# victordeleau/MUI-DeepAutoEncoder

Hardware: AMD Instinct MI355X
Metric: training samples/sec at 3x512-dim input, batch 8192 (higher is better)
Workload: dtype bf16; 1 GPU; embedding.yaml topology: 3 slots x 512 (io 1536), z=io, 4+4 layers -> 10 x Linear(1536,1536); batch 8192 rows per GPU, Adam lr 1e-5 wd 1e-4 clip 1.0, slot-blanking k=1; global_batch=8192, parallelism=dp1

## Files before the change

include/codae_hip.h:

```cpp
#ifndef CODAE_HIP_H
#define CODAE_HIP_H

#include <stddef.h>
#include <stdint.h>

#ifdef __cplusplus
extern "C" {
#endif

#define CODAE_ABI_VERSION 11

enum {
    CODAE_OK = 0,
    CODAE_E_INVALID = -1,
    CODAE_E_HIP = -2,
    CODAE_E_UNSUPPORTED = -3
};

enum {
    CODAE_PREC_F32 = 0,
    CODAE_PREC_BF16 = 1
};

enum {
// ... 150 lines not shown
    float max_grad_norm;
    int32_t step;
    float loss_scale_rows;
} codae_hyper;

const char* codae_last_error(void);
int codae_abi_version(void);
#define CODAE_N_STRUCTS 7
int codae_struct_sizes(int32_t* out, int32_t capacity);
int codae_reload_env(void);

int codae_create(const codae_spec* spec, codae_handle* out);
int codae_destroy(codae_handle h);
int codae_get_sizes(codae_handle h, codae_sizes* out);
int codae_param_offsets(codae_handle h, int32_t layer, int64_t* w_off, int64_t* b_off, int64_t* shadow_off);

int codae_forward(codae_handle h, const codae_buffers* bufs, const float* x, float* y, int32_t B,
                  int32_t layer_lo, int32_t layer_hi, int32_t save_for_backward, void* stream);
int codae_backward(codae_handle h, const codae_buffers* bufs, const float* dy, float* dx, int32_t B,
                   int32_t layer_lo, int32_t layer_hi, void* stream);
int codae_sync_shadows(codae_handle h, const codae_buffers* bufs, void* stream);

int codae_step_forward_loss(codae_handle h, const codae_buffers* bufs, const codae_batch* batch,
                            const codae_hyper* hyper, float* out_y, void* stream);
int codae_step_backward(codae_handle h, const codae_buffers* bufs, int32_t B, int32_t layer_lo,
                        int32_t layer_hi, void* stream);
int codae_step_update(codae_handle h, const codae_buffers* bufs, const codae_hyper* hyper, void* stream);
int codae_train_step_graph(codae_handle h, const codae_buffers* bufs, const codae_batch* batch,
                           const codae_hyper* hyper, void* stream);
int codae_step_backward_async(codae_handle h, const codae_buffers* bufs, int32_t B, int32_t layer_lo,
                              int32_t layer_hi, void* stream);
int codae_side_stream(codae_handle h, void** stream_out);
int codae_join(codae_handle h, void* stream);

int codae_span_sumsq(const float* g, int64_t n, double* acc, void* stream);
int codae_step_update_span(codae_handle h, const codae_buffers* bufs, const codae_hyper* hyper, int64_t lo, int64_t hi,
                           const double* total_sq, void* stream);
int codae_sync_transposed(codae_handle h, const codae_buffers* bufs, void* stream);
int codae_train_step(codae_handle h, const codae_buffers* bufs, const codae_batch* batch,
                     const codae_hyper* hyper, void* stream);
int codae_dp_unique_id(void* out, int32_t capacity);
int codae_dp_init(codae_handle h, const void* unique_id, int32_t rank, int32_t world);
int codae_dp_destroy(codae_handle h);
int codae_train_step_dp(codae_handle h, const codae_buffers* bufs, const codae_batch* batch, const codae_hyper* hyper,
                        int32_t n_buckets, const int32_t* bucket_lo, const int32_t* bucket_hi, void* stream);
int codae_step_path(codae_handle h, const codae_buffers* bufs, int32_t B);
int codae_set_input_noise(codae_handle h, const codae_noise* noise);
int codae_set_loss_emphasis(codae_handle h, const codae_emphasis* emphasis);
int codae_set_recon_loss(codae_handle h, const codae_recon_loss* loss);
int codae_set_hidden_dropout(codae_handle h, const codae_dropout* d);
int codae_set_slot_contrast(codae_handle h, const codae_slot_contrast* contrast);
int codae_set_optimizer(codae_handle h, const codae_optimizer* opt);
int codae_set_slot_presence(codae_handle h, const uint8_t* present, int64_t n_rows, int32_t n_slots);
int codae_set_tied_weights(codae_handle h, int32_t on);
int codae_graph_captures(codae_handle h);
int codae_eval_step(codae_handle h, const codae_buffers* bufs, const codae_batch* batch, float* out_y,
                    void* stream);

enum {
    CODAE_K_GEMM_FWD = 0,
    CODAE_K_GEMM_DGRAD = 1,
    CODAE_K_GEMM_WGRAD = 2,
    CODAE_K_LOSS = 3,
    CODAE_K_GATHER = 4,
    CODAE_K_SUMSQ = 5,
    CODAE_K_ADAM = 6,
    CODAE_K_SLAB_REDUCE = 7,
    CODAE_K_CHAIN = 8,
    CODAE_K_BIAS_FINISH = 9,
    CODAE_K_DROPOUT = 10,
    CODAE_K_COUNT = 11
};
int codae_profile_begin(codae_handle h, uint32_t class_mask, int32_t max_records);
int codae_profile_stride(codae_handle h, int32_t every_n_steps);
int codae_profile_end(codae_handle h, int32_t* kinds, float* ms, int32_t capacity, int32_t* n_out);

int codae_corrupt(const float* x, const float* mask, float* out, int64_t n, void* stream);
int codae_corrupt_batch(const codae_batch* batch, const codae_noise* noise, int32_t step, const int32_t* noise_rows, void* out,
                        int32_t out_bf16, int64_t out_ld, void* stream);
int codae_emph_loss(const codae_batch* batch, const codae_noise* noise, int32_t step, const codae_emphasis* emphasis, const float* y,
                    void* dy, int32_t dy_bf16, int64_t dy_ld, float inv_n, float* colsum_part, double* parts, void* stream);
int codae_emph_loss_blocks(int32_t B);
int codae_recon_loss_fwd_bwd(const codae_batch* batch, const codae_noise* noise, int32_t step, const codae_emphasis* emphasis,
                             const codae_recon_loss* loss, const float* y, void* dy, int32_t dy_bf16, int64_t dy_ld, float inv_n,
                             float* colsum_part, double* parts, void* stream);
int codae_recon_loss_blocks(int32_t B);
int64_t codae_slot_contrast_ws_bytes(int32_t n_slots, int32_t n_neg, int32_t E, int32_t bf16);
int codae_slot_contrast_prepare(const float* data, int32_t io, const codae_slot_contrast* contrast, int32_t step, int32_t bf16, void* stream);
int codae_slot_contrast_fwd_bwd(const codae_batch* batch, const codae_noise* noise, int32_t step, const codae_emphasis* emphasis,
                                const codae_slot_contrast* contrast, const float* y, void* dy, int32_t dy_bf16, int64_t dy_ld, float scale,
                                float* colsum_part, double* parts, void* stream);
int codae_slot_contrast_blocks(int32_t B);
int codae_corrupt_batch_present(const codae_batch* batch, const codae_noise* noise, int32_t step, const int32_t* noise_rows, void* out,
                                int32_t out_bf16, int64_t out_ld, const uint8_t* present, int32_t n_slots, void* stream);
int codae_mse_loss_present(const codae_batch* batch, const float* y, void* dy, int32_t dy_bf16, int64_t dy_ld, float inv_n,
                           float* colsum_part, double* parts, const uint8_t* present, int32_t n_slots, void* stream);
int codae_emph_loss_present(const codae_batch* batch, const codae_noise* noise, int32_t step, const codae_emphasis* emphasis, const float* y,
                            void* dy, int32_t dy_bf16, int64_t dy_ld, float inv_n, float* colsum_part, double* parts,
                            const uint8_t* present, int32_t n_slots, void* stream);
int codae_recon_loss_fwd_bwd_present(const codae_batch* batch, const codae_noise* noise, int32_t step, const codae_emphasis* emphasis,
                                     const codae_recon_loss* loss, const float* y, void* dy, int32_t dy_bf16, int64_t dy_ld, float inv_n,
                                     float* colsum_part, double* parts, const uint8_t* present, int32_t n_slots, void* stream);
int codae_slot_contrast_prepare_present(const float* data, int32_t io, const codae_slot_contrast* contrast, int32_t step, int32_t bf16,
                                        const uint8_t* present, int32_t n_slots, void* stream);
int codae_slot_contrast_fwd_bwd_present(const codae_batch* batch, const codae_noise* noise, int32_t step, const codae_emphasis* emphasis,
                                        const codae_slot_contrast* contrast, const float* y, void* dy, int32_t dy_bf16, int64_t dy_ld,
// ... 26 lines not shown
                             const int32_t* var_size, const int32_t* var_type, const float* undo_scale, const float* undo_min,
                             const int32_t* mask_id, const uint8_t* mask_table, const int32_t* k_of_mask, int32_t k_max,
                             double* acc, void* stream);
int codae_row_norms(const float* m, int64_t rows, int32_t E, float* out, void* stream);
int codae_ranking_loss(const float* pred, const float* fmask, const int32_t* idx, int32_t B, int32_t io, int32_t n_slots,
                       int32_t E, const float* inventory, const float* inventory_norm, int64_t n_obs, const int32_t* val_idx,
                       int32_t n_val, double* out, void* stream);

int codae_ranking_loss_batched(const float* pred, int32_t B, int32_t io, int32_t n_slots, int32_t E, const int32_t* row_idx,
                               const int32_t* mask_id, const int32_t* mask_to_use, int32_t nb_run, int32_t run,
                               const uint8_t* mask_table, const float* inventory, const float* inventory_norm, int64_t n_obs,
                               const float* inv_val, const float* inv_val_norm, const int32_t* val_pos, const int32_t* val_group,
                               int32_t n_val, float* work, int32_t chunk, void* row_state, int32_t* perm_ws, float* q_ws, double* out,
                               void* stream);
int codae_gather_inventory_rows(const float* inventory, int64_t n_obs, int32_t E, int32_t n_slots, const int32_t* val_idx,
                                int32_t n_val, float* dst, void* stream);

int codae_topk_init(void* state, int32_t B, int32_t k, void* stream);
int codae_topk_merge(const float* scores, int64_t ld, int32_t rows, int32_t n, int32_t col0, int32_t k, const int32_t* row_map,
                     const int32_t* skip_col, void* state, void* stream);
int codae_topk_finish(const void* state, int32_t B, int32_t k, const int32_t* cand_row_id, int32_t* out_idx, float* out_score,
                      void* stream);
int codae_complete_topk(const float* pred, int32_t B, int32_t io, int32_t n_slots, int32_t E, const int32_t* slot,
                        const int32_t* row_idx, const int32_t* mask_id, const int32_t* mask_to_use, int32_t nb_run, int32_t run,
                        const uint8_t* mask_table, const float* cand, const float* cand_norm, const int32_t* cand_row_id,
                        int32_t n_cand, const int32_t* cand_count, const int32_t* exclude, const int32_t* cand_pos, int64_t n_obs,
                        int32_t k, float* work, int32_t chunk, void* row_state, int32_t* perm_ws, float* q_ws, void* topk_state,
                        int32_t* out_idx, float* out_score, void* stream);

int codae_linear_f32(const float* x, const float* W, const float* b, float* y, int32_t M, int32_t N,
                     int32_t K, int32_t relu, void* stream);
int codae_dgrad_f32(const float* dy, const float* W, const float* relu_src, float* dx, int32_t M,
                    int32_t N, int32_t K, void* stream);
int codae_wgrad_f32(const float* dy, const float* x, float* dW, float* db, int32_t M, int32_t N,
                    int32_t K, void* stream);
int codae_linear_bf16(const void* x, const void* W, const float* b, void* y, int32_t y_f32, int32_t M,
                      int32_t N, int32_t K, int32_t relu, void* stream);
int codae_dgrad_bf16(const void* dy, const void* W, const void* relu_src, void* dx, float* db_prev, float* db_ws,
                     int32_t M, int32_t N, int32_t K, void* stream);
int codae_wgrad_bf16(const void* dy, const void* x, float* dW, void* slabs, int64_t slab_bytes,
                     int32_t M, int32_t N, int32_t K, void* stream);
int codae_linear_act_f32(const float* x, const float* W, const float* b, float* y, int32_t M, int32_t N, int32_t K,
                         int32_t act, float p0, float p1, float p2, void* stream);
int codae_dgrad_act_f32(const float* dy, const float* W, const float* act_src, float* dx, int32_t M, int32_t N, int32_t K,
                        int32_t act, float p0, float p1, float p2, void* stream);
int codae_linear_act_bf16(const void* x, const void* W, const float* b, void* y, int32_t y_f32, int32_t M, int32_t N,
                          int32_t K, int32_t act, float p0, float p1, float p2, void* stream);
int codae_dgrad_act_bf16(const void* dy, const void* W, const void* act_src, void* dx, float* db_prev, float* db_ws,
                         int32_t M, int32_t N, int32_t K, int32_t act, float p0, float p1, float p2, void* stream);
int codae_debug_gemm_timeline(uint64_t* host_out, int32_t n_wg);
#define CODAE_GEMM_PLAN_FIELDS 15
int codae_debug_gemm_bf16_plan(const int32_t* desc, int32_t* out, int32_t capacity);
int codae_cast_f32_to_bf16(const float* src, void* dst, int64_t n, void* stream);
int codae_transpose_bf16(const void* src, void* dst, int32_t rows, int32_t cols, void* stream);

#ifdef __cplusplus
}
#endif
#endif
```

mui-deepautoencoder_amd/codae/hip/__init__.py:

```python
import ctypes as C
import os

_HERE = os.path.dirname(os.path.abspath(__file__))
LIB_PATH = os.environ.get("CODAE_HIP_LIB") or os.path.join(_HERE, "libcodae_hip.so")

PREC_F32 = 0
PREC_BF16 = 1

ABI_VERSION = 11
S_SQ_FULL, S_SQ_PARTIAL, S_GRAD_SQ, S_LAST_LOSS, S_STEP_SQ, S_CLIP_COEF = 0, 1, 2, 3, 4, 5
S_GRAD_SQ_SLOTS, S_N_SLOTS, S_ADAM_STEP, S_COUNT = 8, 64, 72, 80
ACT_NONE, ACT_RELU, ACT_LEAKY, ACT_RELU6, ACT_ELU, ACT_SOFTPLUS, ACT_HARDSIGMOID = 0, 1, 2, 3, 4, 5, 6
NOISE_NONE, NOISE_GAUSSIAN, NOISE_MASKING, NOISE_SALT_PEPPER = 0, 1, 2, 3
LOSS_MSE, LOSS_L1, LOSS_SMOOTH_L1, LOSS_HUBER, LOSS_SLOT_COSINE = 0, 1, 2, 3, 4
OPT_ADAM, OPT_ADAMW, OPT_SGD = 0, 1, 2
SCHED_CONSTANT, SCHED_COSINE, SCHED_LINEAR, SCHED_STEP = 0, 1, 2, 3
KERNEL_CLASSES = ("gemm_fwd", "gemm_dgrad", "gemm_wgrad", "loss", "gather", "sumsq", "adam", "slab_reduce", "chain",
                  "bias_finish", "dropout")


class HipError(RuntimeError):
    pass


# ... 53 lines not shown

class Optimizer(C.Structure):
    _fields_ = [("kind", C.c_int32), ("amsgrad", C.c_int32), ("momentum", C.c_float), ("nesterov", C.c_int32), ("sched", C.c_int32),
                ("warmup", C.c_int32), ("total", C.c_int32), ("period", C.c_int32), ("min_factor", C.c_float), ("gamma", C.c_float),
                ("vmax", C.c_void_p)]


class TiePair(C.Structure):
    _fields_ = [("enc_off", C.c_int64), ("dec_off", C.c_int64), ("rows", C.c_int32), ("cols", C.c_int32)]


class Dropout(C.Structure):
    _fields_ = [("p", C.POINTER(C.c_float)), ("n", C.c_int32), ("seed", C.c_uint64)]


_P, _I32, _I64, _F = C.c_void_p, C.c_int32, C.c_int64, C.c_float

PROTOTYPES = {
    "codae_last_error": (C.c_char_p, []),
    "codae_abi_version": (C.c_int, []),
    "codae_struct_sizes": (C.c_int, [C.POINTER(C.c_int32), _I32]),
    "codae_reload_env": (C.c_int, []),
    "codae_create": (C.c_int, [C.POINTER(Spec), C.POINTER(_P)]),
    "codae_destroy": (C.c_int, [_P]),
    "codae_get_sizes": (C.c_int, [_P, C.POINTER(Sizes)]),
    "codae_param_offsets": (C.c_int, [_P, _I32, C.POINTER(_I64), C.POINTER(_I64), C.POINTER(_I64)]),
    "codae_forward": (C.c_int, [_P, C.POINTER(Buffers), _P, _P, _I32, _I32, _I32, _I32, _P]),
    "codae_backward": (C.c_int, [_P, C.POINTER(Buffers), _P, _P, _I32, _I32, _I32, _P]),
    "codae_sync_shadows": (C.c_int, [_P, C.POINTER(Buffers), _P]),
    "codae_step_forward_loss": (C.c_int, [_P, C.POINTER(Buffers), C.POINTER(Batch), C.POINTER(Hyper), _P, _P]),
    "codae_step_backward": (C.c_int, [_P, C.POINTER(Buffers), _I32, _I32, _I32, _P]),
    "codae_step_update": (C.c_int, [_P, C.POINTER(Buffers), C.POINTER(Hyper), _P]),
    "codae_step_backward_async": (C.c_int, [_P, C.POINTER(Buffers), _I32, _I32, _I32, _P]),
    "codae_side_stream": (C.c_int, [_P, C.POINTER(C.c_void_p)]),
    "codae_profile_stride": (C.c_int, [_P, _I32]),
    "codae_join": (C.c_int, [_P, _P]),
    "codae_span_sumsq": (C.c_int, [_P, _I64, _P, _P]),
    "codae_step_update_span": (C.c_int, [_P, C.POINTER(Buffers), C.POINTER(Hyper), _I64, _I64, _P, _P]),
    "codae_sync_transposed": (C.c_int, [_P, C.POINTER(Buffers), _P]),
    "codae_train_step": (C.c_int, [_P, C.POINTER(Buffers), C.POINTER(Batch), C.POINTER(Hyper), _P]),
    "codae_train_step_graph": (C.c_int, [_P, C.POINTER(Buffers), C.POINTER(Batch), C.POINTER(Hyper), _P]),
    "codae_set_input_noise": (C.c_int, [_P, C.POINTER(Noise)]),
    "codae_set_loss_emphasis": (C.c_int, [_P, C.POINTER(Emphasis)]),
    "codae_set_recon_loss": (C.c_int, [_P, C.POINTER(ReconLoss)]),
    "codae_set_hidden_dropout": (C.c_int, [_P, C.POINTER(Dropout)]),
    "codae_set_slot_contrast": (C.c_int, [_P, C.POINTER(SlotContrast)]),
    "codae_set_optimizer": (C.c_int, [_P, C.POINTER(Optimizer)]),
    "codae_optimizer_update": (C.c_int, [_P, _P, _P, _P, _P, _I64, C.POINTER(Hyper), C.POINTER(Optimizer), _P, _P]),
    "codae_graph_captures": (C.c_int, [_P]),
    "codae_set_tied_weights": (C.c_int, [_P, _I32]),
    "codae_tie_fold": (C.c_int, [_P, C.POINTER(TiePair), _I32, _P]),
    "codae_tie_mirror": (C.c_int, [_P, _P, _P, C.POINTER(TiePair), _I32, _P]),
    "codae_set_slot_presence": (C.c_int, [_P, _P, _I64, _I32]),
    "codae_corrupt_batch_present": (C.c_int, [C.POINTER(Batch), C.POINTER(Noise), _I32, _P, _P, _I32, _I64, _P, _I32, _P]),
    "codae_mse_loss_present": (C.c_int, [C.POINTER(Batch), _P, _P, _I32, _I64, _F, _P, _P, _P, _I32, _P]),
    "codae_emph_loss_present": (C.c_int, [C.POINTER(Batch), C.POINTER(Noise), _I32, C.POINTER(Emphasis), _P, _P, _I32, _I64, _F, _P, _P,
                                          _P, _I32, _P]),
    "codae_recon_loss_fwd_bwd_present": (C.c_int, [C.POINTER(Batch), C.POINTER(Noise), _I32, C.POINTER(Emphasis), C.POINTER(ReconLoss), _P,
                                                   _P, _I32, _I64, _F, _P, _P, _P, _I32, _P]),
    "codae_slot_contrast_prepare_present": (C.c_int, [_P, _I32, C.POINTER(SlotContrast), _I32, _I32, _P, _I32, _P]),
    "codae_slot_contrast_fwd_bwd_present": (C.c_int, [C.POINTER(Batch), C.POINTER(Noise), _I32, C.POINTER(Emphasis),
                                                      C.POINTER(SlotContrast), _P, _P, _I32, _I64, _F, _P, _P, _P, _I32, _P]),
    "codae_slot_contrast_ws_bytes": (_I64, [_I32, _I32, _I32, _I32]),
    "codae_slot_contrast_prepare": (C.c_int, [_P, _I32, C.POINTER(SlotContrast), _I32, _I32, _P]),
    "codae_slot_contrast_fwd_bwd": (C.c_int, [C.POINTER(Batch), C.POINTER(Noise), _I32, C.POINTER(Emphasis), C.POINTER(SlotContrast), _P, _P,
                                              _I32, _I64, _F, _P, _P, _P]),
    "codae_slot_contrast_blocks": (C.c_int, [_I32]),
    "codae_dropout_fwd": (C.c_int, [_P, _I32, _I64, _I32, _I32, _P, _I32, _I32, _F, C.c_uint64, _P]),
    "codae_dropout_bwd": (C.c_int, [_P, _I32, _I64, _I32, _I32, _P, _I32, _I32, _F, C.c_uint64, _P, _P]),
    "codae_dropout_blocks": (C.c_int, [_I32]),
    "codae_emph_loss": (C.c_int, [C.POINTER(Batch), C.POINTER(Noise), _I32, C.POINTER(Emphasis), _P, _P, _I32, _I64, _F, _P, _P, _P]),
    "codae_emph_loss_blocks": (C.c_int, [_I32]),
    "codae_recon_loss_fwd_bwd": (C.c_int, [C.POINTER(Batch), C.POINTER(Noise), _I32, C.POINTER(Emphasis), C.POINTER(ReconLoss), _P, _P, _I32, _I64,
                                           _F, _P, _P, _P]),
    "codae_recon_loss_blocks": (C.c_int, [_I32]),
    "codae_corrupt_batch": (C.c_int, [C.POINTER(Batch), C.POINTER(Noise), _I32, _P, _P, _I32, _I64, _P]),
    "codae_noise_box_muller": (C.c_int, [_P, _P, _P, _P, _P, _I64, _P]),
    "codae_eval_step": (C.c_int, [_P, C.POINTER(Buffers), C.POINTER(Batch), _P, _P]),
    "codae_profile_begin": (C.c_int, [_P, C.c_uint32, _I32]),
    "codae_profile_end": (C.c_int, [_P, C.POINTER(C.c_int32), C.POINTER(C.c_float), _I32, C.POINTER(C.c_int32)]),
    "codae_corrupt": (C.c_int, [_P, _P, _P, _I64, _P]),
    "codae_expand_masks": (C.c_int, [_P, _P, _P, _I32, _I32, _I32, _P, _P, _P]),
    "codae_mse_loss_fwd_bwd": (C.c_int, [_P, _P, _P, _P, _I64, _F, _P, _P]),
    "codae_clip_adam": (C.c_int, [_P, _P, _P, _P, _I64, C.POINTER(Hyper), _P, _P]),
    "codae_combined_loss_fwd_bwd": (C.c_int, [_P, _P, _I32, _I32, _I32, _P, _P, _P, _P, _P, _P, _P, _P]),
    "codae_combined_loss_full": (C.c_int, [_P, _P, _I32, _I32, _I32, _P, _P, _P, _P, _P]),
    "codae_row_norms": (C.c_int, [_P, _I64, _I32, _P, _P]),
    "codae_ranking_loss": (C.c_int, [_P, _P, _P, _I32, _I32, _I32, _I32, _P, _P, _I64, _P, _I32, _P, _P]),
    "codae_ranking_loss_batched": (C.c_int, [_P, _I32, _I32, _I32, _I32, _P, _P, _P, _I32, _I32, _P, _P, _P, _I64, _P, _P, _P, _P, _I32, _P,
                                             _I32, _P, _P, _P, _P, _P]),
    "codae_dp_unique_id": (C.c_int, [_P, _I32]),
    "codae_dp_init": (C.c_int, [_P, _P, _I32, _I32]),
    "codae_dp_destroy": (C.c_int, [_P]),
    "codae_train_step_dp": (C.c_int, [_P, C.POINTER(Buffers), C.POINTER(Batch), C.POINTER(Hyper), _I32, _P, _P, _P]),
    "codae_monitor_accumulate": (C.c_int, [_P, _P, _I32, _I32, _I32, _P, _P, _P, _P, _P, _P, _P, _P, _I32, _P, _P]),
    "codae_gather_inventory_rows": (C.c_int, [_P, _I64, _I32, _I32, _P, _I32, _P, _P]),
    "codae_topk_init": (C.c_int, [_P, _I32, _I32, _P]),
    "codae_topk_merge": (C.c_int, [_P, _I64, _I32, _I32, _I32, _I32, _P, _P, _P, _P]),
    "codae_topk_finish": (C.c_int, [_P, _I32, _I32, _P, _P, _P, _P]),
    "codae_complete_topk": (C.c_int, [_P, _I32, _I32, _I32, _I32, _P, _P, _P, _P, _I32, _I32, _P, _P, _P, _P, _I32, _P, _P, _P, _I64,
                                      _I32, _P, _I32, _P, _P, _P, _P, _P, _P, _P]),
    "codae_step_path": (C.c_int, [_P, _P, _I32]),
    "codae_linear_f32": (C.c_int, [_P, _P, _P, _P, _I32, _I32, _I32, _I32, _P]),
    "codae_dgrad_f32": (C.c_int, [_P, _P, _P, _P, _I32, _I32, _I32, _P]),
    "codae_wgrad_f32": (C.c_int, [_P, _P, _P, _P, _I32, _I32, _I32, _P]),
    "codae_linear_bf16": (C.c_int, [_P, _P, _P, _P, _I32, _I32, _I32, _I32, _I32, _P]),
    "codae_dgrad_bf16": (C.c_int, [_P, _P, _P, _P, _P, _P, _I32, _I32, _I32, _P]),
    "codae_wgrad_bf16": (C.c_int, [_P, _P, _P, _P, _I64, _I32, _I32, _I32, _P]),
    "codae_linear_act_f32": (C.c_int, [_P, _P, _P, _P, _I32, _I32, _I32, _I32, _F, _F, _F, _P]),
    "codae_dgrad_act_f32": (C.c_int, [_P, _P, _P, _P, _I32, _I32, _I32, _I32, _F, _F, _F, _P]),
    "codae_linear_act_bf16": (C.c_int, [_P, _P, _P, _P, _I32, _I32, _I32, _I32, _I32, _F, _F, _F, _P]),
    "codae_dgrad_act_bf16": (C.c_int, [_P, _P, _P, _P, _P, _P, _I32, _I32, _I32, _I32, _F, _F, _F, _P]),
    "codae_cast_f32_to_bf16": (C.c_int, [_P, _P, _I64, _P]),
    "codae_debug_gemm_timeline": (C.c_int, [_P, _I32]),
    "codae_debug_gemm_bf16_plan": (C.c_int, [_P, _P, _I32]),
    "codae_transpose_bf16": (C.c_int, [_P, _P, _I32, _I32, _P]),
}

_lib = None


def lib():
    global _lib
    if _lib is not None:
        return _lib
    if not os.path.exists(LIB_PATH):
        raise HipError(
            "libcodae_hip.so is missing (%s). Build it with `python -c \"import __graft_entry__ as g; "
            "g.build()\"` or `make -C mui-deepautoencoder_amd/csrc`. There is no CPU fallback." % LIB_PATH)
    import torch
    handle = C.CDLL(LIB_PATH, mode=C.RTLD_GLOBAL)
    for name, (res, args) in PROTOTYPES.items():
        fn = getattr(handle, name)
        fn.restype = res
        fn.argtypes = args
    if handle.codae_abi_version() != ABI_VERSION:
        raise HipError("libcodae_hip.so ABI version %d, this binding is written for %d: rebuild the library"
                       % (handle.codae_abi_version(), ABI_VERSION))
    check_struct_sizes(handle)
    _lib = handle
    return _lib


def struct_sizes_expected():
    return [C.sizeof(Spec), C.sizeof(Sizes), C.sizeof(Buffers), C.sizeof(Batch), C.sizeof(Hyper), S_COUNT,
            len(KERNEL_CLASSES)]


def check_struct_sizes(handle):
    n = 7
    got = (C.c_int32 * n)()
    rc = handle.codae_struct_sizes(got, n)
    if rc != 0:
        raise HipError("codae_struct_sizes failed (%d)" % rc)
    want = struct_sizes_expected()
    names = ("codae_spec", "codae_sizes", "codae_buffers", "codae_batch", "codae_hyper", "CODAE_S_COUNT", "CODAE_K_COUNT")
    bad = ["%s: library %d, binding %d" % (nm, g, w) for nm, g, w in zip(names, list(got), want) if g != w]
    if bad:
        raise HipError("libcodae_hip.so and its ctypes binding disagree: " + "; ".join(bad))


def check(rc):
    if rc != 0:
        msg = lib().codae_last_error()
        raise HipError("codae_hip error %d: %s" % (rc, msg.decode() if msg else "?"))

# ... 9 lines not shown
```

mui-deepautoencoder_amd/codae/hip/engine.py:

```python
import ctypes as C

import torch

from . import (PREC_BF16, PREC_F32, S_COUNT, S_GRAD_SQ, S_GRAD_SQ_SLOTS, S_LAST_LOSS, S_N_SLOTS, S_SQ_FULL, S_SQ_PARTIAL,
               Batch, Buffers, Dropout, Emphasis,
               HipError, Hyper, Sizes, Spec, TiePair, check, current_stream, lib, ptr)


def precision_code(precision):
    if precision in (PREC_F32, "f32", "fp32", "parity"):
        return PREC_F32
    if precision in (PREC_BF16, "bf16", "throughput"):
        return PREC_BF16
    raise ValueError("unknown precision %r (use 'f32' or 'bf16')" % (precision,))


def _tie_pair_array(pairs):
    arr = (TiePair * max(len(pairs), 1))()
    for i, (e, d, r, c) in enumerate(pairs):
        arr[i] = TiePair(int(e), int(d), int(r), int(c))
    return arr


def tie_fold(grads, pairs):
# ... 28 lines not shown
        self.max_batch = int(max_batch)
        self.precision = precision_code(precision)
        ins = (C.c_int32 * self.L)(*[s[0] for s in self.schedule])
        outs = (C.c_int32 * self.L)(*[s[1] for s in self.schedule])
        relu = (C.c_uint8 * self.L)(*[1 if s[2] else 0 for s in self.schedule])
        self.activation = self._layer_acts(activation)
        spec = Spec(self.L, ins, outs, relu, self.max_batch, self.precision)
        if self.activation is not None:
            spec.act_kind = (C.c_uint8 * self.L)(*[a[0] for a in self.activation])
            spec.act_param = (C.c_float * (3 * self.L))(*[float(p) for a in self.activation for p in a[1:]])
        h = C.c_void_p()
        check(self._lib.codae_create(C.byref(spec), C.byref(h)))
        self._h = h
        sz = Sizes()
        check(self._lib.codae_get_sizes(self._h, C.byref(sz)))
        self.n_param = int(sz.n_param)
        with torch.cuda.device(device):
            f32 = dict(dtype=torch.float32, device=device)
            self._params = torch.zeros(self.n_param, **f32)
            self.grads = torch.zeros(self.n_param, **f32)
            self.adam_m = torch.zeros(self.n_param, **f32) if with_optimizer_state else None
            self.adam_v = torch.zeros(self.n_param, **f32) if with_optimizer_state else None
            self.shadow = (torch.zeros(int(sz.n_weight), dtype=torch.bfloat16, device=device)
                           if sz.n_weight > 0 else None)
            self.shadow_t = (torch.zeros(int(sz.n_weight), dtype=torch.bfloat16, device=device)
                             if sz.n_weight > 0 else None)
            self.acts = torch.zeros(max(int(sz.act_bytes), 16), dtype=torch.uint8, device=device)
            self.dacts = torch.zeros(max(int(sz.dact_bytes), 16), dtype=torch.uint8, device=device)
            self.slabs = (torch.zeros(int(sz.slab_bytes), dtype=torch.uint8, device=device)
                          if sz.slab_bytes > 0 else None)
            self.bias_parts = torch.zeros(max(int(sz.bias_part_bytes) // 4, 16), dtype=torch.float32, device=device)
            if int(sz.n_scalars) != S_COUNT:
                raise HipError("library reports %d scalars, binding expects %d" % (int(sz.n_scalars), S_COUNT))
            self.scalars = torch.zeros(int(sz.n_scalars), dtype=torch.float64, device=device)
        self.bufs = Buffers(ptr(self._params), ptr(self.grads), ptr(self.adam_m), ptr(self.adam_v), ptr(self.shadow),
                            ptr(self.acts), ptr(self.dacts), ptr(self.slabs), ptr(self.scalars), ptr(self.shadow_t),
                            ptr(self.bias_parts))
        self.w_off, self.b_off = [], []
        for l in range(self.L):
            w, b, s = C.c_int64(), C.c_int64(), C.c_int64()
            check(self._lib.codae_param_offsets(self._h, l, C.byref(w), C.byref(b), C.byref(s)))
            self.w_off.append(w.value)
            self.b_off.append(b.value)
        self.input_noise = None
        self.loss_emphasis = None
        self._emph_weights = None
        self.hidden_dropout = None
        self.recon_loss = None
        self.slot_contrast = None
        self._contrast_pins = None
        self.slot_presence = None
        self._presence_table = None
        self.tied_weights = False
        self.optimizer = None
        self.adam_vmax = None
        self.step_count = 0
        self.generation = 0

    def _layer_acts(self, activation):
        if activation is None:
            return None
        if isinstance(activation, (list, tuple)) and len(activation) == self.L and all(
                isinstance(a, (list, tuple)) for a in activation):
            acts = [tuple(a) for a in activation]
        else:
            if isinstance(activation, (list, tuple)):
                one = tuple(activation)
            else:
                from ..model.activation import from_factory
                one = from_factory(activation)
            acts = [one if s[2] else (0, 0.0, 0.0, 0.0) for s in self.schedule]
        for a in acts:
            if len(a) != 4:
                raise HipError("activation per layer must be (kind, p0, p1, p2), got %r" % (a,))
        return [(int(a[0]), float(a[1]), float(a[2]), float(a[3])) for a in acts]

    def __del__(self):
        h = getattr(self, "_h", None)
        if h is not None and h.value:
            try:
                self._lib.codae_destroy(h)
            except Exception:
                pass
            self._h = None

    def join(self):
        with torch.cuda.device(self.device):
            check(self._lib.codae_join(self._h, current_stream()))

    @property
    def params(self):
        self.join()
        return self._params

    def _view(self, flat, l, bias):
        self.join()
        k, n, _ = self.schedule[l]
        if bias:
            return flat[self.b_off[l]:self.b_off[l] + n]
        return flat[self.w_off[l]:self.w_off[l] + n * k].view(n, k)

    def weight(self, l): return self._view(self._params, l, False)
    def bias(self, l): return self._view(self._params, l, True)
    def weight_grad(self, l): return self._view(self.grads, l, False)
    def bias_grad(self, l): return self._view(self.grads, l, True)

# ... 89 lines not shown
    def _set_recon_struct(self, st):
        check(self._lib.codae_set_recon_loss(self._h, None if st is None else C.byref(st)))

    def set_slot_contrast(self, contrast, data=None, n_slots=None):
        if contrast is not None and not hasattr(contrast, "candidate_rows"):
            raise HipError("set_slot_contrast: expected a codae.tool.SlotContrast or None, got %r" % (contrast,))
        if contrast is None or contrast.is_default:
            self._set_contrast_struct(None)
            self.slot_contrast, self._contrast_pins = contrast, None
            return
        if data is None or data.dtype != torch.float32 or not data.is_contiguous() or data.device != self.device or data.dim() != 2:
            raise HipError("set_slot_contrast: data must be the contiguous fp32 [N, io] dataset on %s" % self.device)
        io = self.schedule[-1][1]
        if int(data.shape[1]) != io:
            raise HipError("set_slot_contrast: data has %d columns, the model %d" % (int(data.shape[1]), io))
        S = contrast._check_slots(n_slots, io)
        N = int(data.shape[0])
        contrast.check_rows(N)
        with torch.cuda.device(self.device):
            pool = None if contrast.candidates is None else torch.from_numpy(contrast.candidates).to(self.device)
            ids = None
            if contrast.distinct:
                from ..tool.contrast import item_ids
                ids = item_ids(data, S).to(torch.int32).contiguous()
            need = int(self._lib.codae_slot_contrast_ws_bytes(S, contrast.negatives, io // S, int(self.precision == PREC_BF16)))
            if need < 0:
                raise HipError("set_slot_contrast: no work space for S = %d, K = %d, E = %d" % (S, contrast.negatives, io // S))
            ws = torch.empty(need, dtype=torch.uint8, device=self.device)
        self._set_contrast_struct(contrast.as_struct(S, N, pool, ids, ws))
        self.slot_contrast, self._contrast_pins = contrast, (data, pool, ids, ws)

    def _set_contrast_struct(self, st):
        with torch.cuda.device(self.device):
            check(self._lib.codae_set_slot_contrast(self._h, None if st is None else C.byref(st)))

    def set_slot_presence(self, presence):
        if presence is not None and not hasattr(presence, "assign_masks"):
            raise HipError("set_slot_presence: expected a codae.tool.SlotPresence or None, got %r" % (presence,))
        if presence is None or presence.is_default:
            self._set_presence_table(None)
            self.slot_presence, self._presence_table = presence, None
            return
        table = presence.to(self.device)
        self._set_presence_table(table)
        self.slot_presence, self._presence_table = presence, table

    def _set_presence_table(self, table, n_rows=None, n_slots=None):
        if table is None:
            check(self._lib.codae_set_slot_presence(self._h, None, 0, 0))
            return
        check(self._lib.codae_set_slot_presence(self._h, ptr(table), int(table.shape[0]) if n_rows is None else int(n_rows),
                                                int(table.shape[1]) if n_slots is None else int(n_slots)))

    def set_optimizer(self, optimizer):
        if optimizer is not None and not hasattr(optimizer, "lr_at"):
            raise HipError("set_optimizer: expected a codae.tool.Optimizer or None, got %r" % (optimizer,))
        if optimizer is None or optimizer.is_default:
            self._set_optimizer_struct(None)
            self.optimizer = optimizer
            return
        vmax = self.adam_vmax
        if optimizer.amsgrad and vmax is None:
            with torch.cuda.device(self.device):
                vmax = torch.zeros(self.n_param, dtype=torch.float32, device=self.device)
        self._set_optimizer_struct(optimizer.as_struct(ptr(vmax)))
        self.optimizer, self.adam_vmax = optimizer, vmax

    def _set_optimizer_struct(self, st):
        check(self._lib.codae_set_optimizer(self._h, None if st is None else C.byref(st)))

    def set_tied_weights(self, on):
        on = bool(on)
        check(self._lib.codae_set_tied_weights(self._h, 1 if on else 0))
        self.tied_weights = on
        if on:
            self.sync_shadows()

    def tie_pairs(self):
        from ..tool.tied import TiedWeights
        return TiedWeights.flat_pairs(self.schedule, self.w_off)

    def graph_captures(self):
        return int(self._lib.codae_graph_captures(self._h))

    def set_hidden_dropout(self, dropout):
        if dropout is not None and not hasattr(dropout, "per_layer"):
            raise HipError("set_hidden_dropout: expected a codae.tool.HiddenDropout or None, got %r" % (dropout,))
        self._set_dropout_values(None if dropout is None else dropout.per_layer(self.L), 0 if dropout is None else dropout.seed)
        self.hidden_dropout = dropout

    def _set_dropout_values(self, p, seed=0):
        st = None
        if p is not None:
            arr = (C.c_float * max(len(p), 1))(*[float(v) for v in p])
            st = Dropout(arr, len(p), int(seed))
        check(self._lib.codae_set_hidden_dropout(self._h, None if st is None else C.byref(st)))

    def train_step(self, batch, hyper, graph=False):
        fn = self._lib.codae_train_step_graph if graph else self._lib.codae_train_step
        with torch.cuda.device(self.device):
            check(fn(self._h, C.byref(self.bufs), C.byref(batch), C.byref(hyper), current_stream()))
        self.step_count += 1

    def dp_unique_id(self):
        buf = (C.c_char * 128)()
        check(self._lib.codae_dp_unique_id(buf, 128))
# ... 104 lines not shown
```

mui-deepautoencoder_amd/codae/train.py:

```python
import torch

from .hostcpu import fit_host_threads, host_cpu_share
from .hip import HipError


class SubsetEpochSampler:

    def __init__(self, indices, batch_size):
        self.indices = torch.as_tensor(list(indices), dtype=torch.long)
        self.batch_size = int(batch_size)

    def __len__(self):
        return (len(self.indices) + self.batch_size - 1) // self.batch_size

    def _epoch_order(self):
        torch.empty((), dtype=torch.int64).random_()
        n_threads = torch.get_num_threads()
        if n_threads > 1:
            torch.set_num_threads(1)
        try:
            perm = torch.randperm(len(self.indices))
        finally:
            if n_threads > 1:
                torch.set_num_threads(n_threads)
        return self.indices[perm]

    def __iter__(self):
        order = self._epoch_order()
        for o in range(0, len(order), self.batch_size):
            yield order[o:o + self.batch_size]

    def device_batches(self, device, dtype=torch.int32):
        order = self._epoch_order().to(dtype)
        if torch.device(device).type == "cuda":
            st = getattr(self, "_stage", None)
            if st is None or st[0].numel() != order.numel() or st[0].dtype != order.dtype or st[1].device != torch.device(device):
                st = (torch.empty(order.numel(), dtype=order.dtype).pin_memory(), torch.empty(order.numel(), dtype=order.dtype, device=device),
                      torch.cuda.Event())
                self._stage = st
            else:
                st[2].synchronize()
            st[0].copy_(order)
            st[1].copy_(st[0], non_blocking=True)
            st[2].record()
            order = st[1]
        else:
            order = order.to(device)
        for o in range(0, len(order), self.batch_size):
            yield order[o:o + self.batch_size]


def shard_batch(batch_indices, rank, world):
# ... 202 lines not shown
        self.last_grad_sq = acc
        if hasattr(eng, "record_grad_sq"):
            eng.record_grad_sq(acc)
        for lo, hi in self.buckets:
            a, b = self._shard_bounds(lo, hi)
            eng.step_update_span(hyper, a, b, acc)
        eng.step_update_span(hyper, eng.b_off[0], eng.n_param, acc)
        in_place = self.dist.get_backend(self.group) == "nccl"
        works = []
        for t in eng.replica_tensors():
            for lo, hi in self.buckets:
                a, b = self._weight_span_bounds(lo, hi)
                sa, sb = self._shard_bounds(lo, hi)
                src = t[sa:sb] if in_place else t[sa:sb].clone()
                works.append(self.dist.all_gather_into_tensor(t[a:b], src, group=self.group, async_op=True))
        for w in works:
            w.wait()
        eng.after_replica_sync()
        eng.step_count += 1

    def gather_params(self):
        if not self.sharded or self.world == 1:
            return
        eng = self.engine
        p = eng.params if not hasattr(eng, "_params") else eng._params
        for lo, hi in self.buckets:
            a, b = self._weight_span_bounds(lo, hi)
            sa, sb = self._shard_bounds(lo, hi)
            self.dist.all_gather_into_tensor(p[a:b], p[sa:sb].clone(), group=self.group)

    def broadcast_params(self, params_flat):
        if self.world > 1:
            self.dist.broadcast(params_flat, src=0, group=self.group)

    def reduce_scalars(self, t):
        if self.world > 1:
            self.dist.all_reduce(t, op=self.dist.ReduceOp.SUM, group=self.group)
        return t


class _ResidentInventory:

    def __init__(self, data, S, E):
        self.nb_used_category, self.embedding_size = S, E
        self.data_per_category = {c: data[:, c * E:(c + 1) * E] for c in range(S)}


class HipEmbeddingTrainer:

    def __init__(self, schedule, data, mask_table_u8, mask_to_use_i32, lr, weight_decay, clip=1.0,
                 max_batch=8192, precision="bf16", device="cuda:0", distributed=False, n_buckets=None, use_graph=False,
                 sharded_update=False, native_dp=False, activation=None, n_slots=None, input_noise=None,
                 loss_emphasis=None, hidden_dropout=None, criterion=None, contrast=None, optimizer=None, presence=None,
                 tied_weights=None):
        from .hip.engine import DaeEngine
        fit_host_threads()
        self.device = torch.device(device)
        self.engine = DaeEngine(schedule, max_batch, precision, self.device, activation=activation)
        if input_noise is not None:
            self.engine.set_input_noise(input_noise)
        self.data = data.to(device=self.device, dtype=torch.float32).contiguous()
        self.mask_table = None if mask_table_u8 is None else mask_table_u8.to(self.device).contiguous()
        self.mask_to_use = None if mask_to_use_i32 is None else mask_to_use_i32.to(self.device).contiguous()
        self.lr, self.weight_decay, self.clip = lr, weight_decay, clip
        self.n_slots = n_slots
        if loss_emphasis is not None:
            self.set_loss_emphasis(loss_emphasis)
        if hidden_dropout is not None:
            self.set_hidden_dropout(hidden_dropout)
        if criterion is not None:
            self.set_criterion(criterion)
        if contrast is not None:
            self.set_contrast(contrast)
        if optimizer is not None:
            self.set_optimizer(optimizer)
        self.presence = None
        if presence is not None:
            self.set_presence(presence)
        if tied_weights:
            self.set_tied_weights(True)
        self.dp = DataParallel(self.engine, n_buckets=n_buckets, sharded=sharded_update, native=native_dp) if distributed else None
        self.world = self.dp.world if self.dp else 1
        self.use_graph = bool(use_graph) and self.dp is None
        self._idx_buf = torch.zeros(max_batch, dtype=torch.int32, device=self.device) if self.use_graph else None
        self._mid_buf = torch.zeros(max_batch, dtype=torch.int32, device=self.device) if self.use_graph else None
        self._graph_stream = torch.cuda.Stream(device=self.device) if self.use_graph else None

    def set_loss_emphasis(self, emphasis):
        S = None
        if emphasis is not None and getattr(emphasis, "slot_weight", None) is not None and (self.n_slots or self.mask_table is not None):
            S = self._slots()[0]
        self.engine.set_loss_emphasis(emphasis, n_slots=S)

    def set_criterion(self, criterion):
        S = None
        if criterion is not None and getattr(criterion, "kind", None) == "slot_cosine":
            if not self.n_slots and self.mask_table is None:
                raise HipError("criterion slot_cosine: the trainer has neither n_slots nor a mask table to read the slots from; "
                               "construct it with n_slots")
            S = self._slots()[0]
        self.engine.set_recon_loss(criterion, n_slots=S)

    def set_contrast(self, contrast):
        S = None
        if contrast is not None and not getattr(contrast, "is_default", True):
            if not self.n_slots and self.mask_table is None:
                raise HipError("slot contrast: the trainer has neither n_slots nor a mask table to read the slots from; "
                               "construct it with n_slots")
            S = self._slots()[0]
        self.engine.set_slot_contrast(contrast, self.data, n_slots=S)

    def set_presence(self, presence):
        if presence is not None and not getattr(presence, "is_default", True) and presence.n_rows != int(self.data.shape[0]):
            raise HipError("slot presence: the table has %d rows, the dataset %d" % (presence.n_rows, int(self.data.shape[0])))
        self.engine.set_slot_presence(presence)
        self.presence = None if presence is None or presence.is_default else presence
        self.__dict__.pop("_retrievers", None)

    def set_tied_weights(self, on):
        dp = self.__dict__.get("dp")
        if on and dp is not None and dp.sharded and self.engine.L >= 2:
            from .tool.tied import TiedWeights
            raise TiedWeights.sharded_refusal(self.engine.L)
        self.engine.set_tied_weights(bool(on))

    def set_optimizer(self, optimizer):
        self.engine.set_optimizer(optimizer)

    def current_lr(self):
        opt = self.engine.optimizer
        if opt is None:
            from .tool.optimizer import Optimizer
            opt = Optimizer()
        return opt.lr_at(self.lr, self.engine.step_count + 1)

    def set_hidden_dropout(self, dropout):
        self.engine.set_hidden_dropout(dropout)

    def load_params(self, params):
# ... 129 lines not shown
```

mui-deepautoencoder_amd/csrc/codae_common.h:

```cpp
#pragma once
#include <hip/hip_runtime.h>
#include <stdint.h>
#include <stdio.h>
#include <type_traits>

#include "codae_hip.h"

namespace codae {

void set_error(const char* fmt, ...);

#define CODAE_HIP_CHECK(expr)                                                              \
    do {                                                                                   \
        hipError_t e_ = (expr);                                                            \
        if (e_ != hipSuccess) {                                                            \
            codae::set_error("%s failed: %s (%s:%d)", #expr, hipGetErrorString(e_), __FILE__, __LINE__); \
            return CODAE_E_HIP;                                                            \
        }                                                                                  \
    } while (0)

#define CODAE_LAUNCH_CHECK()                                                               \
    do {                                                                                   \
        hipError_t e_ = hipGetLastError();                                                 \
        if (e_ != hipSuccess) {                                                            \
// ... 129 lines not shown
        k0 += 0x9E3779B9u; k1 += 0xBB67AE85u;
    }
    return make_uint4(c0, c1, c2, c3);
}

struct PresArgs {
    const uint8_t* tab;
    int S, E;
};
template <int W>
__device__ __forceinline__ uint32_t present_bits(const PresArgs& p, int64_t row, const int* sl) {
    const uint8_t* __restrict__ t = p.tab + row * p.S;
    const uint32_t p0 = t[sl[0]] != 0 ? 1u : 0u;
    if (sl[W - 1] == sl[0]) return p0 ? ((1u << W) - 1u) : 0u;
    uint32_t bits = p0;
#pragma unroll
    for (int k = 1; k < W; ++k) bits |= (t[sl[k]] != 0 ? 1u : 0u) << k;
    return bits;
}
int check_presence(const uint8_t* present, int n_slots, int io, const char* who);

static inline int64_t round_up(int64_t x, int64_t m) { return (x + m - 1) / m * m; }

enum { STORE_PLAIN = 0, STORE_WT = 1 };
int store_policy_for(int64_t out_bytes);

template <int POL>
struct TileStore {
    __amdgpu_buffer_rsrc_t rsrc;
    __device__ __forceinline__ explicit TileStore(void* tile_base) {
        if constexpr (POL != STORE_PLAIN) rsrc = __builtin_amdgcn_make_buffer_rsrc(tile_base, 0, 0x7fffffff, 0x00020000);
    }
    __device__ __forceinline__ void store16(void* p, uint32_t byte_off, u32x4 v) const {
        if constexpr (POL == STORE_PLAIN) *reinterpret_cast<u32x4*>(p) = v;
        else __builtin_amdgcn_raw_buffer_store_b128(v, rsrc, (int)byte_off, 0, 16);
    }
};

struct EnvToggles {
    int gemm_tile = -1;
    int gemm_dbg = 0;
    int wgrad_splitk = 0;
    int small_tile_max = 200;
    int small_stages = 4;
    int f32_gemm = 0;
    int group_tile = -1;
    bool side_priority_set = false; int side_priority = 0;
    bool no_wt = false, single_stream = false, tail_on_side = false, no_fused_loss = false, flat_adam = false,
         no_fused_norm = false, no_chain = false, no_deep_small = false,
         no_relu_bits = false,
         no_prefetch = false,
         no_defer_wgrad = false;
    bool no_folded_loss_finish = false;
    int store_policy = -1;
};
const EnvToggles& env();
void env_reload();

struct GemmF32 {
    const float* A; int64_t a_rs, a_ks;
    const float* B; int64_t b_rs, b_ks;
    float* C; int64_t ldc;
    int M, N, K;
    const float* bias;
    int relu;
    const float* relu_src;
    int64_t ld_relu;
    float* colsum_part;
    const int* m_dev;
    int split_k;
    int act;
    float act_p[3];
};
int gemm_f32(const GemmF32& g, hipStream_t s);
int gemm_f32x3(const GemmF32& g, hipStream_t s);
bool gemm_f32x3_takes(const GemmF32& g);
inline int gemm_f32_colsum_rows(int M) { return (M + 63) / 64; }

constexpr int CODAE_GROUP_MAX = 16;
struct GemmF32Group {
    int n;
    GemmF32 g[CODAE_GROUP_MAX];
    int wg_begin[CODAE_GROUP_MAX + 1];
};
int gemm_f32x3_grouped(GemmF32Group& grp, hipStream_t s);

enum { OP_KC = 0,
       OP_KS = 1
};
struct LossFuse {
    int enabled;
    const float* data;
    const int32_t* row_idx;
    const int32_t* mask_id;
    const int32_t* mask_to_use;
    int nb_run, run;
    const uint8_t* table;
    int io;
    int B;
    float inv_n;
    double* parts;
};

struct GemmBf16 {
    const bf16_t* A; int64_t lda; int a_mode;
    const bf16_t* B; int64_t ldb; int b_mode;
// ... 1 lines not shown
    int M, N, K;
    const float* bias;
    int relu;
    const bf16_t* relu_src; int64_t ld_relu;
    float* colsum_part;
    int split_k;
    LossFuse loss;
    int dbg;
    uint8_t* relu_bits_out; const uint8_t* relu_bits; int64_t ld_bits;
    const void* prefetch; int64_t prefetch_bytes;
    int coscheduled;
    double* sumsq_slots;
    int act;
    float act_p[3];
    int store_policy;
};
bool gemm_bf16_supported(int M, int N, int K);

struct GemmTile { int bm, bn; };
constexpr GemmTile TILE_256x192{256, 192}, TILE_128x192{128, 192}, TILE_128x128{128, 128}, TILE_64x128{64, 128}, TILE_64x64{64, 64};
inline int ceil_div(int a, int b) { return (a + b - 1) / b; }
inline int tile_count(int M, int N, GemmTile t) { return ceil_div(M, t.bm) * ceil_div(N, t.bn); }

enum { BF16_ONE_BARRIER = 0,
       BF16_PIPELINED = 1,
       BF16_PIPELINED_ABL = 2
};
struct Bf16Plan {
    int family;
    int bm, bn;
    int stages;
    int loader;
    int epi;
    int dbg;
    int act;
    int store_policy;
    int tiles_m, tiles_n;
    int64_t workgroups;
};
Bf16Plan gemm_bf16_plan(const GemmBf16& g);
bool gemm_bf16_takes_relu_bits(int M, int N);
int gemm_bf16_colsum_rows(const GemmBf16& g);
int gemm_bf16_loss_parts(const GemmBf16& g);
int gemm_bf16(const GemmBf16& g, hipStream_t s);
int gemm_bf16_pipe(const GemmBf16& g, const Bf16Plan& plan, hipStream_t s);
int choose_split_k(int N, int K, int rows);

struct GemmBf16Group {
    int n;
    GemmBf16 g[CODAE_GROUP_MAX];
    int wg_begin[CODAE_GROUP_MAX + 1];
};
int gemm_bf16_grouped(GemmBf16Group& grp, hipStream_t s);
int gemm_bf16_pipe_grouped(GemmBf16Group& grp, hipStream_t s);

constexpr int CODAE_CHAIN_MAX_WIDTH = 512;
constexpr int CODAE_CHAIN_MAX_LAYERS = 16;
constexpr int CODAE_CHAIN_MAX_BIAS = 6144;
struct ChainArgs {
    int L, rows, B;
    int width[CODAE_CHAIN_MAX_LAYERS + 1];
    uint32_t relu_flags;
    double* scalars;
    const bf16_t* W[CODAE_CHAIN_MAX_LAYERS];
    const bf16_t* Wt[CODAE_CHAIN_MAX_LAYERS];
    const float* bias[CODAE_CHAIN_MAX_LAYERS];
    bf16_t* act[CODAE_CHAIN_MAX_LAYERS];
    bf16_t* dact[CODAE_CHAIN_MAX_LAYERS];
    float* colsum_part[CODAE_CHAIN_MAX_LAYERS];
    const float* data; const int32_t* row_idx; const int32_t* mask_id; const uint8_t* mask_table;
    const int32_t* mask_to_use; int nb_run, run;
    float inv_n;
    double* loss_parts;
    int do_backward;
};
bool chain_supported(int L, const int* in, const int* out);
int chain_rows_per_workgroup();
int launch_chain_step(const ChainArgs& a, hipStream_t s);

int launch_gather_corrupt(const codae_batch* b, void* out, int out_bf16, hipStream_t s, int64_t out_ld = 0, double* zero_norm = nullptr,
                          const uint8_t* present = nullptr, int n_slots = 0);
int check_noise(const codae_noise* noise);
int launch_gather_noise(const codae_batch* b, const codae_noise* noise, int32_t step, const double* step_dev, void* out,
                        int out_bf16, hipStream_t s, int64_t out_ld = 0, const int32_t* noise_rows = nullptr, double* zero_norm = nullptr,
                        const uint8_t* present = nullptr, int n_slots = 0);
int launch_noise_box_muller(const uint32_t* ra, const uint32_t* rb, float* rho, float* c, float* sn, int64_t n, hipStream_t s);
int launch_cast_bf16(const float* src, bf16_t* dst, int64_t n, hipStream_t s);
int launch_corrupt(const float* x, const float* mask, float* out, int64_t n, hipStream_t s);
int launch_expand_masks(const int32_t* mask_id, const uint8_t* table, const int32_t* k_of_mask, int B, int io,
                        int k_max, float* masks_out, float* fmask_out, hipStream_t s);
struct LossLaunch {
    const codae_batch* batch; const codae_noise* noise; int32_t step; const double* step_dev;
    const codae_emphasis* emph; const uint8_t* present; int n_slots;
    const float* y; void* dy; int dy_bf16; int64_t dy_ld; float scale ;
    float* colsum_part; double* parts;
};
inline int64_t loss_dy_ld(const LossLaunch& ll) { return ll.dy_ld > 0 ? ll.dy_ld : (ll.batch ? ll.batch->io : 0); }
int check_loss_launch(const char* who, const LossLaunch& ll, bool needs_dy);
int launch_mse_loss(const LossLaunch& ll, int want_grad, hipStream_t s);
int mse_loss_colsum_rows(int B);
int check_emphasis(const codae_emphasis* emph);
int launch_emph_loss(const LossLaunch& ll, hipStream_t s);
int launch_finish_emph_loss(double* scalars, double inv_n, hipStream_t s, const double* parts, int n_parts);
int check_recon_loss(const codae_recon_loss* loss, int io);
int launch_recon_loss(const LossLaunch& ll, const codae_recon_loss* loss, hipStream_t s);
int check_slot_contrast(const codae_slot_contrast* c, int io, int bf16);
int64_t slot_contrast_ws_bytes(int S, int K, int E, int bf16);
inline int slot_contrast_blocks(int B) { return (B + 31) / 32; }
int slot_contrast_warm();
int launch_slot_contrast_prepare(const float* data, int io, const codae_slot_contrast* c, int32_t step, const double* step_dev, int bf16,
                                 hipStream_t s, const uint8_t* present = nullptr, int n_slots = 0);
int launch_slot_contrast(const LossLaunch& ll, const codae_slot_contrast* c, hipStream_t s);
int launch_slot_contrast_finish(double* scalars, double scale, const double* parts, int n_parts, hipStream_t s);
int check_dropout_p(float p, const char* who);
inline int dropout_blocks(int B) { return (B + 63) / 64; }
int launch_dropout_fwd(void* a, int bf16, int64_t ld, int B, int width, const int32_t* row_idx, int layer, int32_t step,
                       const double* step_dev, float p, uint64_t seed, hipStream_t s);
int launch_dropout_bwd(void* d, int bf16, int64_t ld, int B, int width, const int32_t* row_idx, int layer, int32_t step,
                       const double* step_dev, float p, uint64_t seed, float* colsum_part, hipStream_t s);
int launch_mse_dense(const float* x, const float* y, const float* fmask, float* dy, int64_t n, float inv_n,
                     double* scalars, hipStream_t s);
int launch_sumsq(const float* g, int64_t n, double* out, hipStream_t s);
int launch_sumsq_to(const float* g, int64_t n, double* acc, hipStream_t s);
int launch_clip_coef(const double* total_sq, float max_norm, double* coef_out, hipStream_t s);
int launch_clip_adam(float* p, float* g, float* m, float* v, int64_t n, const codae_hyper* hp,
                     const double* grad_sq, bf16_t* shadow, const double* coef_in, hipStream_t s,
                     const double* step_dev = nullptr, const codae_optimizer* opt = nullptr, float* vmax = nullptr);
int check_optimizer(const codae_optimizer* o);
bool optimizer_is_default(const codae_optimizer* o);
codae_optimizer optimizer_canonical(const codae_optimizer* o);
int launch_set_scalar(double* dst, double value, hipStream_t s);
int launch_clip_adam_tiled(float* p, float* g, float* m, float* v, const codae_hyper* hp, const double* grad_sq,
                           bf16_t* shadow, bf16_t* shadow_t, int n_layers, const int64_t* w_off, const int* rows,
                           const int* cols, int transposed_from, int64_t bias_off, int64_t bias_n, hipStream_t s,
                           const double* step_dev = nullptr, const codae_optimizer* opt = nullptr, float* vmax = nullptr);
int launch_tie_fold(float* g, const codae_tie_pair* pairs, int n, hipStream_t s);
int launch_tie_mirror(float* p, bf16_t* shadow, bf16_t* shadow_t, const codae_tie_pair* pairs, int n, hipStream_t s);
int launch_transpose_bf16(const bf16_t* src, bf16_t* dst, int n, const int64_t* off, const int* rows, const int* cols,
                          hipStream_t s);
int gemm_bf16_timeline(unsigned long long* host_out, int n_wg);
int launch_reduce_slabs_epi(const float* slabs, int n_slabs, int64_t stride, int M, int N, float* C, int64_t ldc, const float* bias,
                            int relu, const float* relu_src, int64_t ld_relu, float* colsum_part, hipStream_t s,
                            int act = CODAE_ACT_NONE, const float* act_p = nullptr);
int launch_reduce_slabs(const float* slabs, int n_slabs, int64_t slab_stride, float* out, int64_t n, double* sumsq,
                        hipStream_t s);
int launch_finish_loss(double* scalars, double inv_n, hipStream_t s, const double* parts = nullptr, int n_parts = 0);
int launch_cast_f32(const bf16_t* src, float* dst, int64_t n, hipStream_t s);
int launch_colsum_f32(const float* src, int M, int N, float* out, hipStream_t s);
int launch_colsum_parts_f32(const float* src, int M, int N, float* parts, hipStream_t s);
struct BiasFinishJobs {
    int n;
    const float* parts[64];
    float* out[64];
    int rows[64], cols[64];
    int col_begin[65];
};
struct LossFinish { double* scalars; double inv_n; const double* parts; int n_parts; };
int launch_bias_finish(const BiasFinishJobs& jobs, double* sumsq, hipStream_t s, const LossFinish* loss = nullptr);

}
```

mui-deepautoencoder_amd/csrc/elementwise.hip:

```cpp
#include "loss_sweep.h"

namespace codae {
namespace {

constexpr int NT = 256;
static_assert(NT == LOSS_NT, "loss_sweep strides the columns by LOSS_NT threads");

inline int grid_for(int64_t work_items) {
    int64_t b = (work_items + NT - 1) / NT;
    if (b < 1) b = 1;
    if (b > 2048) b = 2048;
    return (int)b;
}

template <int W>
__device__ __forceinline__ void zero_absent(float* v, const PresArgs& pa, int64_t row, int c) {
    int sl[W];
    slots_of<W>(c, pa.E, sl);
    const uint32_t pb = present_bits<W>(pa, row, sl);
#pragma unroll
    for (int k = 0; k < W; ++k) v[k] = ((pb >> k) & 1u) ? v[k] : 0.f;
}

__device__ __forceinline__ void zero_norm_scalars(double* zero_norm) {
    if (zero_norm != nullptr && blockIdx.x == 0) {
        if (threadIdx.x == 0) zero_norm[CODAE_S_GRAD_SQ] = 0.0;
        if (threadIdx.x < CODAE_S_N_SLOTS) zero_norm[CODAE_S_GRAD_SQ_SLOTS + threadIdx.x] = 0.0;
    }
}

template <bool PRES>
__global__ __launch_bounds__(NT) void gather_corrupt_bf16x8_kernel(const float* __restrict__ data,
                                                                   const int32_t* __restrict__ row_idx,
                                                                   const int32_t* __restrict__ mask_id,
                                                                   const uint8_t* __restrict__ table, int B, int io,
                                                                   bf16_t* __restrict__ out,
                                                                   const int32_t* __restrict__ mask_to_use, int nb_run,
                                                                   int run, int64_t out_ld, double* zero_norm, PresArgs pa) {
    zero_norm_scalars(zero_norm);
    const bool masked = (mask_id != nullptr) || (mask_to_use != nullptr);
    const int cols = io / 8;
    const int64_t total = (int64_t)B * cols;
    for (int64_t e = (int64_t)blockIdx.x * NT + threadIdx.x; e < total; e += (int64_t)gridDim.x * NT) {
        const int b = (int)(e / cols);
        const int c = (int)(e - (int64_t)b * cols) * 8;
        const int64_t src_row = row_idx ? row_idx[b] : b;
        const float* src = data + src_row * io + c;
        const float4 x0 = *reinterpret_cast<const float4*>(src);
        const float4 x1 = *reinterpret_cast<const float4*>(src + 4);
        float v[8] = {x0.x, x0.y, x0.z, x0.w, x1.x, x1.y, x1.z, x1.w};
        if (masked) {
            const int id = mask_id ? mask_id[b] : mask_to_use[src_row * nb_run + run];
            const uint2 m = *reinterpret_cast<const uint2*>(table + (int64_t)id * io + c);
#pragma unroll
            for (int k = 0; k < 8; ++k) v[k] = (((k < 4 ? m.x : m.y) >> (8 * (k & 3))) & 0xff) ? v[k] : 0.f;
        }
        if constexpr (PRES) zero_absent<8>(v, pa, src_row, c);
        uint4 o;
        o.x = pack_bf16x2(v[0], v[1]); o.y = pack_bf16x2(v[2], v[3]);
        o.z = pack_bf16x2(v[4], v[5]); o.w = pack_bf16x2(v[6], v[7]);
        *reinterpret_cast<uint4*>(out + (int64_t)b * out_ld + c) = o;
    }
}

template <bool VEC, bool OUT_BF16, bool PRES>
__global__ __launch_bounds__(NT) void gather_corrupt_kernel(const float* __restrict__ data,
                                                            const int32_t* __restrict__ row_idx,
                                                            const int32_t* __restrict__ mask_id,
                                                            const uint8_t* __restrict__ table, int B, int io,
                                                            void* __restrict__ out,
                                                            const int32_t* __restrict__ mask_to_use, int nb_run,
                                                            int run, int64_t out_ld, double* zero_norm, PresArgs pa) {
    zero_norm_scalars(zero_norm);
    constexpr int W = VEC ? 4 : 1;
    const bool masked = (mask_id != nullptr) || (mask_to_use != nullptr);
    const int cols = io / W;
    const int64_t total = (int64_t)B * cols;
    for (int64_t e = (int64_t)blockIdx.x * NT + threadIdx.x; e < total; e += (int64_t)gridDim.x * NT) {
        const int b = (int)(e / cols);
        const int c = (int)(e - (int64_t)b * cols) * W;
        const int64_t src_row = row_idx ? row_idx[b] : b;
        const float* src = data + src_row * io + c;
        float v[4];
        if constexpr (VEC) {
            const float4 x = *reinterpret_cast<const float4*>(src);
            v[0] = x.x; v[1] = x.y; v[2] = x.z; v[3] = x.w;
            if (masked) {
                const int id = mask_id ? mask_id[b] : mask_to_use[src_row * nb_run + run];
                const uint32_t m = *reinterpret_cast<const uint32_t*>(table + (int64_t)id * io + c);
#pragma unroll
                for (int k = 0; k < 4; ++k) v[k] = ((m >> (8 * k)) & 0xff) ? v[k] : 0.f;
            }
        } else {
            v[0] = src[0];
            if (masked) {
                const int id = mask_id ? mask_id[b] : mask_to_use[src_row * nb_run + run];
                v[0] = table[(int64_t)id * io + c] ? v[0] : 0.f;
            }
        }
        if constexpr (PRES) zero_absent<W>(v, pa, src_row, c);
        const int64_t o = (int64_t)b * out_ld + c;
        if constexpr (OUT_BF16) {
            bf16_t* op = reinterpret_cast<bf16_t*>(out) + o;
            if constexpr (VEC) *reinterpret_cast<uint2*>(op) = pack_bf16x4(v[0], v[1], v[2], v[3]);
            else op[0] = f32_to_bf16(v[0]);
        } else {
            float* op = reinterpret_cast<float*>(out) + o;
            if constexpr (VEC) *reinterpret_cast<float4*>(op) = make_float4(v[0], v[1], v[2], v[3]);
            else op[0] = v[0];
        }
    }
}

// ... 660 lines not shown
        if (c0 + c < C && r0 + r8 < R) {
            bf16_t e[8];
#pragma unroll
            for (int k = 0; k < 8; ++k) e[k] = tile[r8 + k][c];
            uint4 v;
            v.x = (uint32_t)e[0] | ((uint32_t)e[1] << 16); v.y = (uint32_t)e[2] | ((uint32_t)e[3] << 16);
            v.z = (uint32_t)e[4] | ((uint32_t)e[5] << 16); v.w = (uint32_t)e[6] | ((uint32_t)e[7] << 16);
            *reinterpret_cast<uint4*>(D + (int64_t)(c0 + c) * R + r0 + r8) = v;
        }
    }
}

}

int check_presence(const uint8_t* present, int n_slots, int io, const char* who) {
    if (present == nullptr) return CODAE_OK;
    CODAE_REQUIRE(n_slots >= 1 && n_slots <= 128, "%s: slot presence takes 1 .. 128 slots, got %d", who, n_slots);
    CODAE_REQUIRE(io > 0 && io % n_slots == 0, "%s: slot presence: n_slots %d does not divide io %d", who, n_slots, io);
    return CODAE_OK;
}

int launch_gather_corrupt(const codae_batch* b, void* out, int out_bf16, hipStream_t s, int64_t out_ld, double* zero_norm,
                          const uint8_t* present, int n_slots) {
    if (out_ld <= 0) out_ld = b ? b->io : 0;
    CODAE_REQUIRE(b && b->data && out && b->B > 0 && b->io > 0, "gather_corrupt: bad batch");
    int prc = check_presence(present, n_slots, b->io, "gather_corrupt");
    if (prc) return prc;
    const PresArgs pa{present, n_slots, present ? b->io / n_slots : 0};
    const bool masked = b->mask_id || b->mask_to_use;
    CODAE_REQUIRE(!masked || b->mask_table, "gather_corrupt: mask ids without mask_table");
    CODAE_REQUIRE(!b->mask_to_use || b->mask_id || (b->nb_run > 0 && b->run >= 0 && b->run < b->nb_run),
                  "gather_corrupt: run %d outside [0, %d)", b->run, b->nb_run);
    const bool vec = (b->io % 4 == 0) && (out_ld % 4 == 0) && a16(b->data) && a16(out) && (!masked || (reinterpret_cast<uintptr_t>(b->mask_table) & 3) == 0);
    const int64_t items = (int64_t)b->B * (vec ? b->io / 4 : b->io);
    const int grid = grid_for(items);
    if (vec && out_bf16 && b->io % 8 == 0 && (!masked || (reinterpret_cast<uintptr_t>(b->mask_table) & 7) == 0)) {
#define GC8(P) hipLaunchKernelGGL((gather_corrupt_bf16x8_kernel<P>), dim3(grid_for(items / 2)), dim3(NT), 0, s, b->data, b->row_idx, b->mask_id, \
                                  b->mask_table, b->B, b->io, reinterpret_cast<bf16_t*>(out), b->mask_to_use, b->nb_run, b->run, out_ld, zero_norm, pa)
        if (present) GC8(true);
        else GC8(false);
#undef GC8
        CODAE_LAUNCH_CHECK();
        return CODAE_OK;
    }
#define GCP(V, O, P) hipLaunchKernelGGL((gather_corrupt_kernel<V, O, P>), dim3(grid), dim3(NT), 0, s, b->data, b->row_idx, \
                                    b->mask_id, b->mask_table, b->B, b->io, out, b->mask_to_use, b->nb_run, b->run, out_ld, zero_norm, pa)
#define GC(V, O) do { if (present) GCP(V, O, true); else GCP(V, O, false); } while (0)
    if (vec && out_bf16) GC(true, true);
    else if (vec) GC(true, false);
    else if (out_bf16) GC(false, true);
    else GC(false, false);
#undef GC
#undef GCP
    CODAE_LAUNCH_CHECK();
    return CODAE_OK;
}

int check_noise(const codae_noise* n) {
    if (n == nullptr || n->kind == CODAE_NOISE_NONE) return CODAE_OK;
    CODAE_REQUIRE(n->kind == CODAE_NOISE_GAUSSIAN || n->kind == CODAE_NOISE_MASKING || n->kind == CODAE_NOISE_SALT_PEPPER,
                  "input noise: unknown kind %d", n->kind);
    if (n->kind == CODAE_NOISE_GAUSSIAN) {
        CODAE_REQUIRE(finite_f(n->p0) && n->p0 >= 0.f, "input noise: sigma %g must be finite and >= 0", (double)n->p0);
        return CODAE_OK;
    }
    CODAE_REQUIRE(finite_f(n->p0) && n->p0 >= 0.f && n->p0 <= 1.f, "input noise: p %g outside [0, 1]", (double)n->p0);
    if (n->kind == CODAE_NOISE_SALT_PEPPER) {
        CODAE_REQUIRE(finite_f(n->p1), "input noise: lo %g is not finite", (double)n->p1);
        CODAE_REQUIRE(finite_f(n->p2), "input noise: hi %g is not finite", (double)n->p2);
    }
    return CODAE_OK;
}

int launch_gather_noise(const codae_batch* b, const codae_noise* noise, int32_t step, const double* step_dev, void* out, int out_bf16,
                        hipStream_t s, int64_t out_ld, const int32_t* noise_rows, double* zero_norm, const uint8_t* present, int n_slots) {
    if (noise == nullptr || noise->kind == CODAE_NOISE_NONE) {
        CODAE_REQUIRE(present == nullptr || noise_rows == nullptr, "gather_corrupt: a presence table with noise_rows needs an input noise kind");
        return launch_gather_corrupt(b, out, out_bf16, s, out_ld, zero_norm, present, n_slots);
    }
    int rc = check_noise(noise);
    if (rc) return rc;
    rc = check_presence(present, n_slots, b ? b->io : 0, "gather_corrupt");
    if (rc) return rc;
    const PresArgs pa{present, n_slots, present ? b->io / n_slots : 0};
    if (out_ld <= 0) out_ld = b ? b->io : 0;
    CODAE_REQUIRE(b && b->data && out && b->B > 0 && b->io > 0, "gather_corrupt: bad batch");
    const bool masked = b->mask_id || b->mask_to_use;
    CODAE_REQUIRE(!masked || b->mask_table, "gather_corrupt: mask ids without mask_table");
    CODAE_REQUIRE(!b->mask_to_use || b->mask_id || (b->nb_run > 0 && b->run >= 0 && b->run < b->nb_run),
                  "gather_corrupt: run %d outside [0, %d)", b->run, b->nb_run);
    NoiseArgs na{};
    na.key0 = (uint32_t)(noise->seed & 0xffffffffu); na.key1 = (uint32_t)(noise->seed >> 32);
    na.step = (uint32_t)step; na.step_dev = step_dev; na.rows = noise_rows; na.zero_norm = zero_norm;
    na.thresh = (uint64_t)floor((double)noise->p0 * 4294967296.0);
    na.p0 = noise->p0; na.p1 = noise->p1; na.p2 = noise->p2;
    const bool vec = (b->io % 4 == 0) && (out_ld % 4 == 0) && a16(b->data) && a16(out) && (!masked || (reinterpret_cast<uintptr_t>(b->mask_table) & 3) == 0);
    const int64_t items = (int64_t)b->B * (vec ? b->io / 4 : b->io);
    const int grid = grid_for(items);
    const bool x8 = vec && out_bf16 && b->io % 8 == 0 && (!masked || (reinterpret_cast<uintptr_t>(b->mask_table) & 7) == 0);
#define GN8P(K, P) hipLaunchKernelGGL((gather_noise_bf16x8_kernel<K, P>), dim3(grid_for(items / 2)), dim3(NT), 0, s, b->data, b->row_idx, b->mask_id, \
                                  b->mask_table, b->B, b->io, reinterpret_cast<bf16_t*>(out), b->mask_to_use, b->nb_run, b->run, out_ld, na, pa)
#define GNP(V, O, K, P) hipLaunchKernelGGL((gather_noise_kernel<V, O, K, P>), dim3(grid), dim3(NT), 0, s, b->data, b->row_idx, b->mask_id, \
                                       b->mask_table, b->B, b->io, out, b->mask_to_use, b->nb_run, b->run, out_ld, na, pa)
#define GN8(K) do { if (present) GN8P(K, true); else GN8P(K, false); } while (0)
#define GN(V, O, K) do { if (present) GNP(V, O, K, true); else GNP(V, O, K, false); } while (0)
#define GN_KIND(K)                           \
// ... 468 lines not shown
```

mui-deepautoencoder_amd/csrc/engine.hip:

```cpp
#include <stdarg.h>
#include <stdlib.h>
#include <string.h>

#include <cmath>
#include <vector>

#include "layer_gemm.h"
#include <dlfcn.h>
#include <rccl/rccl.h>

namespace codae {

static thread_local char g_err[512] = "";

void set_error(const char* fmt, ...) {
    va_list ap;
    va_start(ap, fmt);
    vsnprintf(g_err, sizeof(g_err), fmt, ap);
    va_end(ap);
}

static EnvToggles g_env;
static bool g_env_loaded = false;

void env_reload() {
    EnvToggles e;
    if (const char* t = getenv("CODAE_GEMM_TILE")) {
        switch (t[0]) { case 's': e.gemm_tile = 0; break; case 'q': e.gemm_tile = 3; break; case 'x': e.gemm_tile = 6; break; case 'm': e.gemm_tile = 7; break; default: break; }
    }
    if (const char* d = getenv("CODAE_GEMM_DBG")) e.gemm_dbg = atoi(d);
    if (const char* k = getenv("CODAE_WGRAD_SPLITK")) e.wgrad_splitk = atoi(k) > 0 ? atoi(k) : 0;
    if (const char* k = getenv("CODAE_GROUP_TILE")) e.group_tile = (k[0] >= '0' && k[0] <= '2') ? k[0] - '0' : -1;
    if (const char* pr = getenv("CODAE_SIDE_PRIORITY")) { e.side_priority_set = true; e.side_priority = atoi(pr); }
    e.no_wt = getenv("CODAE_NO_WT") != nullptr;
    e.single_stream = getenv("CODAE_SINGLE_STREAM") != nullptr;
    e.tail_on_side = getenv("CODAE_TAIL_ON_SIDE") != nullptr;
    e.no_fused_loss = getenv("CODAE_NO_FUSED_LOSS") != nullptr;
    e.flat_adam = getenv("CODAE_FLAT_ADAM") != nullptr;
    e.no_fused_norm = getenv("CODAE_NO_FUSED_NORM") != nullptr;
    e.no_chain = getenv("CODAE_NO_CHAIN") != nullptr;
    e.no_deep_small = getenv("CODAE_NO_DEEP_SMALL") != nullptr;
    e.no_defer_wgrad = getenv("CODAE_NO_DEFER_WGRAD") != nullptr;
    e.no_prefetch = getenv("CODAE_NO_PREFETCH") != nullptr;
    e.no_relu_bits = getenv("CODAE_NO_RELU_BITS") != nullptr;
    e.no_folded_loss_finish = getenv("CODAE_NO_FOLDED_LOSS_FINISH") != nullptr;
    if (const char* k = getenv("CODAE_STORE_POLICY"))
        e.store_policy = !strcmp(k, "plain") ? STORE_PLAIN : (!strcmp(k, "wt") ? STORE_WT : -1);
    if (const char* k = getenv("CODAE_F32_GEMM")) e.f32_gemm = k[0] == 'n' ? 1 : (k[0] == 'x' ? 2 : 0);
    if (const char* k = getenv("CODAE_SMALL_TILE_MAX")) e.small_tile_max = atoi(k);
    if (const char* k = getenv("CODAE_SMALL_STAGES")) e.small_stages = atoi(k) == 2 ? 2 : 4;
    g_env = e;
    g_env_loaded = true;
}

const EnvToggles& env() {
    if (!g_env_loaded) env_reload();
    return g_env;
}

}

using namespace codae;

constexpr int CODAE_MAX_DACT = 16;

struct codae_engine {
    int L = 0;
    std::vector<int> in, out;
    std::vector<int> in_ld, out_ld;
    std::vector<uint8_t> relu;
    std::vector<uint8_t> act;
    std::vector<float> act_p;
    int max_batch = 0, max_rows = 0;
    int prec = CODAE_PREC_F32;
    std::vector<int64_t> w_off, b_off;
    int64_t n_param = 0, bias_begin = 0;
    int maxw = 0;
    std::vector<int64_t> act_off;
    int64_t act_bytes = 0, dact_one = 0, slab_bytes = 0;
    std::vector<int64_t> bits_off;
    int n_dact = 3;
    std::vector<int> split_k;
    std::vector<int64_t> part_off;
    int64_t part_floats = 0;
    int64_t loss_part_off = 0;
    int loss_part_cap = 0;
    bool chain_ok = false;
    struct PresCfg { const uint8_t* table; int64_t n_rows; int32_t n_slots; int32_t reserved; };
    struct DropCfg { float p[64]; uint64_t seed; int32_t on; int32_t reserved; };
    struct TrainCfg {
        codae_noise noise;
        codae_emphasis emph;
        int32_t emph_on, reserved;
        codae_recon_loss recon;
        codae_slot_contrast contrast;
        PresCfg pres;
        DropCfg drop;
        codae_optimizer opt;
        int32_t tied, tied_reserved;
    } tc;
    bool recon_on() const { return tc.recon.kind != CODAE_LOSS_MSE; }
    bool contrast_on() const { return tc.contrast.weight != 0.f; }
    int n_free() const { return (L + 1) / 2; }
    std::vector<codae_tie_pair> tie_pairs;
    bool plain_mse() const { return !tc.emph_on && !recon_on() && !contrast_on() && tc.pres.table == nullptr; }
    int graph_captures = 0;
    bool drop_live = false;
    int drop_B = 0;
    const int32_t* drop_rows = nullptr;
    int32_t drop_step = 0;
    std::vector<int> parts_pending;
    hipStream_t side = nullptr;
    hipEvent_t ev_ready[CODAE_MAX_DACT] = {}, ev_join = nullptr, ev_w[CODAE_MAX_DACT] = {};
    unsigned ready_turn = 0;
    bool w_pending[CODAE_MAX_DACT] = {};
    bool side_dirty = false;
    bool norm_scalars_zero = false;
    bool prof_on = false;
    uint32_t prof_mask = 0;
    int prof_n = 0;
    int prof_every = 1, prof_step = 0;
    hipGraphExec_t graph_exec = nullptr;
    bool capturing = false;
    struct GraphKey { codae_batch batch; codae_hyper hyper; codae_buffers bufs; TrainCfg tc; } graph_key{};
    std::vector<hipEvent_t> prof_start, prof_stop;
    std::vector<int> prof_kind;
    std::vector<int> prof_count;
    bool prof_group = false;
    EnvToggles cfg;
    struct DpState* dp = nullptr;
    int esize() const { return prec == CODAE_PREC_BF16 ? 2 : 4; }
    int rows_for(int B) const { return prec == CODAE_PREC_BF16 ? (int)round_up(B, 64) : B; }
};

struct RcclApi {
    void* lib = nullptr;
    ncclResult_t (*GetUniqueId)(ncclUniqueId*) = nullptr;
    ncclResult_t (*CommInitRank)(ncclComm_t*, int, ncclUniqueId, int) = nullptr;
    ncclResult_t (*CommDestroy)(ncclComm_t) = nullptr;
    ncclResult_t (*AllReduce)(const void*, void*, size_t, ncclDataType_t, ncclRedOp_t, ncclComm_t, hipStream_t) = nullptr;
    const char* (*GetErrorString)(ncclResult_t) = nullptr;
};
static RcclApi g_rccl;

static int rccl_load() {
    if (g_rccl.lib != nullptr) return CODAE_OK;
    void* lib = nullptr;
    for (const char* name : {"librccl.so.1", "librccl.so"}) {
        lib = dlopen(name, RTLD_NOW | RTLD_NOLOAD | RTLD_LOCAL);
        if (lib != nullptr) break;
    }
    if (lib == nullptr)
// ... 28 lines not shown

constexpr int CODAE_DP_MAX_BUCKETS = 64;
struct DpState {
    ncclComm_t comm = nullptr;
    int rank = 0, world = 1;
    hipStream_t stream = nullptr;
    hipEvent_t ev_bucket[CODAE_DP_MAX_BUCKETS + 1] = {};
    hipEvent_t ev_done = nullptr;
};

namespace {

struct ProfScope {
    codae_engine* e;
    hipStream_t s;
    int slot = -1;
    ProfScope(codae_engine* e_, int kind, hipStream_t s_) : e(e_), s(s_) {
        if (e->prof_group && kind == CODAE_K_GEMM_FWD) return;
        if (e->prof_on && ((e->prof_mask >> kind) & 1u) && (e->prof_step % e->prof_every) == 0 &&
            e->prof_n < (int)e->prof_start.size()) {
            slot = e->prof_n++;
            e->prof_kind[slot] = kind;
            e->prof_count[slot] = 1;
            (void)hipEventRecord(e->prof_start[slot], s);
        }
    }
    void counts_as(int n) { if (slot >= 0) e->prof_count[slot] = n; }
    ~ProfScope() {
        if (slot >= 0) (void)hipEventRecord(e->prof_stop[slot], s);
    }
};

struct GroupScope {
    codae_engine* e;
    hipStream_t s;
    int slot = -1;
    GroupScope(codae_engine* e_, int kind, hipStream_t s_) : e(e_), s(s_) {
        if (e->prof_on && ((e->prof_mask >> kind) & 1u) && (e->prof_step % e->prof_every) == 0 &&
            e->prof_n < (int)e->prof_start.size()) {
            slot = e->prof_n++;
            e->prof_kind[slot] = kind;
            e->prof_count[slot] = 0;
            e->prof_group = true;
            (void)hipEventRecord(e->prof_start[slot], s);
        }
    }
    void launched() { if (slot >= 0) ++e->prof_count[slot]; }
    void close() {
        if (slot >= 0) { (void)hipEventRecord(e->prof_stop[slot], s); e->prof_group = false; slot = -1; }
    }
    ~GroupScope() { close(); }
};

int choose_split_k_f32(int N, int K, int rows) {
    if (env().wgrad_splitk > 0) return env().wgrad_splitk <= rows / 32 ? env().wgrad_splitk : 1;
    if (rows <= 1024) return 1;
    const int tiles = tile_count(N, K, TILE_128x128);
    if (env().f32_gemm != 1 && N % 4 == 0 && K % 4 == 0) {
        int best = 1;
        double best_fill = 0.0;
        for (int s = 1; s <= 8 && s <= rows / 256; ++s) {
            const int wgs = tiles * s, rounds = ceil_div(wgs, 256);
            const double fill = (double)wgs / (256.0 * rounds);
            if (fill > best_fill + 0.02) { best_fill = fill; best = s; }
        }
        return best;
    }
    int s = (384 + tiles / 2) / tiles;
    if (s > 8) s = 8;
    if (s > rows / 256) s = rows / 256;
    return s < 1 ? 1 : s;
}

inline void* act_ptr(codae_engine* e, const codae_buffers* b, int l) {
    return reinterpret_cast<char*>(b->acts) + e->act_off[l];
}
inline float* part_ptr(codae_engine* e, const codae_buffers* b, int l) { return b->bias_parts + e->part_off[l]; }
inline double* loss_parts_ptr(codae_engine* e, const codae_buffers* b) {
    return reinterpret_cast<double*>(b->bias_parts + e->loss_part_off);
}
inline void* dact_ptr(codae_engine* e, const codae_buffers* b, int l) {
    return reinterpret_cast<char*>(b->dacts) + (int64_t)(l % e->n_dact) * e->dact_one;
}

double loss_inv_n(const codae_hyper* hyper, const codae_batch* batch) {
    const float rows = hyper != nullptr && hyper->loss_scale_rows > 0.f ? hyper->loss_scale_rows : (float)batch->B;
    return 1.0 / ((double)rows * batch->io);
}

int finish_loss(codae_engine* e, const codae_buffers* b, const codae_batch* batch, int parts, hipStream_t s) {
    return launch_finish_loss(b->scalars, 1.0 / ((double)batch->B * batch->io), s, loss_parts_ptr(e, b), parts);
}

GemmBf16 layer_fwd_bf16(codae_engine* e, const codae_buffers* b, int l, const void* x, void* y, int64_t ldy, bool y_f32, int rows) {
    return fwd_gemm_bf16(x, e->in_ld[l], reinterpret_cast<const bf16_t*>(b->shadow_w) + e->w_off[l], e->in[l], y, ldy, y_f32 ? 1 : 0, rows,
                         e->out[l], e->in_ld[l], b->params + e->b_off[l]);
}
GemmBf16 layer_wgrad_bf16(codae_engine* e, const codae_buffers* b, int l, int rows) {
    return wgrad_gemm_bf16(dact_ptr(e, b, l), e->out_ld[l], act_ptr(e, b, l), e->in_ld[l], b->grads + e->w_off[l], rows, e->out[l], e->in[l]);
}
GemmF32 layer_wgrad_f32(codae_engine* e, const codae_buffers* b, int l, int rows) {
    return wgrad_gemm_f32(reinterpret_cast<const float*>(dact_ptr(e, b, l)), reinterpret_cast<const float*>(act_ptr(e, b, l)),
                          b->grads + e->w_off[l], rows, e->out[l], e->in[l]);
}

int check_common(codae_handle h, const codae_buffers* b, int B) {
// ... 79 lines not shown
    return finish_loss(e, b, batch, n_wg, s);
}

int run_wgrad_grouped(codae_engine* e, const codae_buffers* b, int rows, bool with_norm, hipStream_t s) {
    for (int base = 0; base < e->L; base += CODAE_GROUP_MAX) {
        GemmBf16Group grp{};
        grp.n = 0;
        for (int l = base; l < e->L && grp.n < CODAE_GROUP_MAX; ++l) {
            GemmBf16& g = grp.g[grp.n++];
            g = layer_wgrad_bf16(e, b, l, rows);
            g.sumsq_slots = with_norm ? b->scalars + CODAE_S_GRAD_SQ_SLOTS : nullptr;
        }
        ProfScope prof(e, CODAE_K_GEMM_WGRAD, s);
        int rc = gemm_bf16_grouped(grp, s);
        if (rc) return rc;
    }
    return CODAE_OK;
}

int defer_wgrad_mode(codae_engine* e, int rows) {
    if (e->prec == CODAE_PREC_F32) {
        if (env().f32_gemm == 1 || e->cfg.no_defer_wgrad || e->cfg.single_stream || e->L > CODAE_GROUP_MAX || e->n_dact <= e->L || rows < 256 ||
            rows % 32 != 0)
            return 0;
        int total = 0;
        for (int l = 0; l < e->L; ++l) {
            if (e->in[l] % 4 != 0 || e->out[l] % 4 != 0) return 0;
            total += tile_count(e->out[l], e->in[l], TILE_128x128);
        }
        return total >= 256 ? 3 : 0;
    }
    if (e->prec != CODAE_PREC_BF16 || e->cfg.no_defer_wgrad || e->cfg.single_stream || e->L > CODAE_GROUP_MAX || e->n_dact <= e->L || rows < 64)
        return 0;
    int total = 0, total_small = 0;
    for (int l = 0; l < e->L; ++l) {
        total += tile_count(e->out[l], e->in[l], TILE_256x192);
        total_small += tile_count(e->out[l], e->in[l], TILE_64x64);
        if ((int64_t)rows * e->out_ld[l] * 2 >= (int64_t)1 << 32 || (int64_t)rows * e->in_ld[l] * 2 >= (int64_t)1 << 32) return 0;
    }
    if (total >= 200) return 1;
    return total_small >= 128 ? 2 : 0;
}

int run_wgrad_deferred_f32(codae_engine* e, const codae_buffers* b, int rows, hipStream_t s) {
    GemmF32Group grp{};
    grp.n = 0;
    for (int l = e->L - 1; l >= 0; --l)
        grp.g[grp.n++] = layer_wgrad_f32(e, b, l, rows);
    ProfScope prof(e, CODAE_K_GEMM_WGRAD, s);
    prof.counts_as(grp.n);
    return gemm_f32x3_grouped(grp, s);
}

int run_wgrad_deferred(codae_engine* e, const codae_buffers* b, int rows, bool with_norm, hipStream_t s) {
    GemmBf16Group grp{};
    grp.n = 0;
    for (int l = e->L - 1; l >= 0; --l) {
        GemmBf16& g = grp.g[grp.n++];
        g = layer_wgrad_bf16(e, b, l, rows);
        g.sumsq_slots = with_norm ? b->scalars + CODAE_S_GRAD_SQ_SLOTS : nullptr;
    }
    ProfScope prof(e, CODAE_K_GEMM_WGRAD, s);
    prof.counts_as(grp.n);
    return gemm_bf16_pipe_grouped(grp, s);
}

int gemm_f32_small(codae_engine* e, const codae_buffers* b, const GemmF32& g, hipStream_t s) {
    const int tiles = tile_count(g.M, g.N, TILE_128x128);
    const int kt = (g.K + 31) / 32;
    int S = tiles >= 128 ? 1 : (256 + tiles / 2) / tiles;
    if (S > kt / 4) S = kt / 4;
    if (S > 16) S = 16;
    while (S > 1 && (int64_t)S * g.M * g.N * 4 > e->slab_bytes) --S;
    if (S <= 1 || b->slabs == nullptr || e->cfg.no_deep_small || (g.N % 4) != 0 || (g.ldc % 4) != 0 || g.m_dev != nullptr ||
        (g.relu_src != nullptr && (g.ld_relu % 4) != 0))
        return gemm_f32(g, s);
    float* slab = reinterpret_cast<float*>(reinterpret_cast<char*>(b->slabs) + 2 * e->slab_bytes);
    GemmF32 p = g;
    p.C = slab; p.ldc = g.N; p.bias = nullptr; p.relu = 0; p.relu_src = nullptr; p.ld_relu = 0; p.colsum_part = nullptr; p.split_k = S;
    p.act = CODAE_ACT_NONE;
    int rc = gemm_f32(p, s);
    if (rc) return rc;
    return launch_reduce_slabs_epi(slab, S, (int64_t)g.M * g.N, g.M, g.N, g.C, g.ldc, g.bias, g.relu, g.relu_src, g.ld_relu, g.colsum_part, s,
                                   g.act, g.act_p);
}

int run_linear(codae_engine* e, const codae_buffers* b, int l, const void* x, void* y, bool y_f32, int rows,
               hipStream_t s) {
    const int N = e->out[l], K = e->in[l];
    ProfScope prof(e, CODAE_K_GEMM_FWD, s);
    if (e->prec == CODAE_PREC_BF16) {
        GemmBf16 g = layer_fwd_bf16(e, b, l, x, y, y_f32 ? N : e->out_ld[l], y_f32, rows);
        set_activation(g, e->relu[l], e->act[l], &e->act_p[3 * l]);
        if (!y_f32 && l + 1 < e->L && e->bits_off[l + 1] >= 0 && e->relu[l] && y == act_ptr(e, b, l + 1) && gemm_bf16_takes_relu_bits(rows, N)) {
            g.relu_bits_out = reinterpret_cast<uint8_t*>(b->acts) + e->bits_off[l + 1];
            g.ld_bits = e->in_ld[l + 1] / 8;
        }
        if (l + 1 < e->L && !e->cfg.no_prefetch) {
            g.prefetch = reinterpret_cast<const bf16_t*>(b->shadow_w) + e->w_off[l + 1];
            g.prefetch_bytes = (int64_t)e->in[l + 1] * e->out[l + 1] * 2;
        }
        return gemm_bf16(g, s);
    }
    GemmF32 g = fwd_gemm_f32(reinterpret_cast<const float*>(x), b->params + e->w_off[l], reinterpret_cast<float*>(y), rows, N, K,
                             b->params + e->b_off[l]);
    set_activation(g, e->relu[l], e->act[l], &e->act_p[3 * l]);
    return gemm_f32_small(e, b, g, s);
}

int run_wgrad(codae_engine* e, const codae_buffers* b, int l, int rows, bool with_norm, hipStream_t s, int slot = 0) {
    const int N = e->out[l], K = e->in[l];
    float* dW = b->grads + e->w_off[l];
    if (e->prec == CODAE_PREC_BF16) {
        const int S = e->split_k[l] <= rows / 64 ? e->split_k[l] : rows / 64;
        GemmBf16 g = layer_wgrad_bf16(e, b, l, rows);
        g.split_k = S;
        if (S > 1) {
// ... 109 lines not shown
        int rc = launch_transpose_bf16(reinterpret_cast<const bf16_t*>(b->shadow_w), reinterpret_cast<bf16_t*>(b->shadow_wt),
                                       n, off, rows, cols, s);
        if (rc) return rc;
    }
    return CODAE_OK;
}

int zero_pad_rows(codae_engine* e, void* base, int B, int rows, int width, hipStream_t s) {
    if (rows > B) {
        char* p = reinterpret_cast<char*>(base) + (int64_t)B * width * e->esize();
        CODAE_HIP_CHECK(hipMemsetAsync(p, 0, (int64_t)(rows - B) * width * e->esize(), s));
    }
    return CODAE_OK;
}

int ensure_side_stream(codae_engine* h) {
    if (h->side != nullptr) return CODAE_OK;
    int prio_least = 0, prio_greatest = 0;
    CODAE_HIP_CHECK(hipDeviceGetStreamPriorityRange(&prio_least, &prio_greatest));
    const int prio = h->cfg.side_priority_set ? h->cfg.side_priority : prio_least;
    CODAE_HIP_CHECK(hipStreamCreateWithPriority(&h->side, hipStreamNonBlocking, prio));
    for (int i = 0; i < CODAE_MAX_DACT; ++i) CODAE_HIP_CHECK(hipEventCreateWithFlags(&h->ev_ready[i], hipEventDisableTiming));
    CODAE_HIP_CHECK(hipEventCreateWithFlags(&h->ev_join, hipEventDisableTiming));
    for (int i = 0; i < CODAE_MAX_DACT; ++i) CODAE_HIP_CHECK(hipEventCreateWithFlags(&h->ev_w[i], hipEventDisableTiming));
    return CODAE_OK;
}

int join_side(codae_engine* h, hipStream_t s) {
    if (!h->side_dirty || h->side == nullptr) return CODAE_OK;
    CODAE_HIP_CHECK(hipEventRecord(h->ev_join, h->side));
    CODAE_HIP_CHECK(hipStreamWaitEvent(s, h->ev_join, 0));
    for (int i = 0; i < CODAE_MAX_DACT; ++i) h->w_pending[i] = false;
    h->side_dirty = false;
    return CODAE_OK;
}

int backward_range(codae_handle h, const codae_buffers* b, int B, int lo, int hi, float* dx, bool step_mode, bool with_norm,
                   hipStream_t s, bool join = true, const LossFinish* loss = nullptr) {
    const int rows = h->rows_for(B);
    const bool dual = !h->cfg.single_stream;
    CODAE_REQUIRE(!(step_mode && h->drop_live && h->tc.drop.on) || B == h->drop_B, "backward of %d rows after a dropped forward of %d", B, h->drop_B);
    if (dual) {
        int rc = ensure_side_stream(h);
        if (rc) return rc;
    }
    const int defer = ((step_mode || dx == nullptr) && join && lo == 0 && hi == h->L && h->L >= 2) ? defer_wgrad_mode(h, rows) : 0;
    if (defer != 0) {
        int rc = join_side(h, s);
        if (rc) return rc;
        for (int l = hi - 1; l >= 1; --l) {
            rc = run_dgrad(h, b, l, rows, false, nullptr, s);
            if (rc) return rc;
        }
        rc = defer == 3 ? run_wgrad_deferred_f32(h, b, rows, s)
                        : (defer == 1 ? run_wgrad_deferred(h, b, rows, with_norm, s) : run_wgrad_grouped(h, b, rows, with_norm, s));
        if (rc) return rc;
        return finish_bias(h, b, s, with_norm, loss);
    }
    bool* w_pending = h->w_pending;
    const bool coscheduled = dual;
    for (int l = hi - 1; l >= lo; --l) {
        int rc;
        if (!dual) {
            rc = run_wgrad(h, b, l, rows, with_norm, s);
        } else if (join && step_mode && l == 0 && hi - lo >= 3 && !h->cfg.tail_on_side) {
            rc = run_wgrad(h, b, l, rows, with_norm, s, 2);
        } else {
            hipEvent_t ready = h->ev_ready[h->ready_turn++ % CODAE_MAX_DACT];
            CODAE_HIP_CHECK(hipEventRecord(ready, s));
            CODAE_HIP_CHECK(hipStreamWaitEvent(h->side, ready, 0));
            rc = run_wgrad(h, b, l, rows, with_norm, h->side, l & 1);
            if (rc == CODAE_OK && h->n_dact <= h->L) {
                CODAE_HIP_CHECK(hipEventRecord(h->ev_w[l % h->n_dact], h->side));
                w_pending[l % h->n_dact] = true;
            }
        }
        if (rc) return rc;
        const bool chain = step_mode ? (l > 0) : (l > lo);
        const bool to_dx = !chain && !step_mode && dx != nullptr;
        if (chain || to_dx) {
            const int wb = (l - 1 + h->n_dact) % h->n_dact;
            if (dual && chain && w_pending[wb]) {
                CODAE_HIP_CHECK(hipStreamWaitEvent(s, h->ev_w[wb], 0));
                w_pending[wb] = false;
            }
            rc = chain ? run_dgrad(h, b, l, rows, coscheduled, nullptr, s) : run_dgrad(h, b, l, B, coscheduled, dx, s);
            if (rc) return rc;
        }
    }
    if (join || lo == 0) {
        int rc = finish_bias(h, b, s, with_norm, loss);
        if (rc) return rc;
    }
    if (dual) {
        h->side_dirty = true;
        if (join) return join_side(h, s);
    }
    return CODAE_OK;
}

}

extern "C" {

const char* codae_last_error(void) { return g_err; }
int codae_abi_version(void) { return CODAE_ABI_VERSION; }

int codae_reload_env(void) {
    env_reload();
// ... 141 lines not shown
    if (e->prec == CODAE_PREC_F32 && e->max_rows <= 512) {
        const int64_t bytes = (int64_t)16 * e->max_rows * e->maxw * 4;
        if (bytes > e->slab_bytes) e->slab_bytes = bytes;
    }
    *out = e;
    return CODAE_OK;
}

static void profile_release(codae_handle h) {
    for (hipEvent_t ev : h->prof_start) (void)hipEventDestroy(ev);
    for (hipEvent_t ev : h->prof_stop) (void)hipEventDestroy(ev);
    h->prof_start.clear(); h->prof_stop.clear(); h->prof_kind.clear(); h->prof_count.clear(); h->prof_group = false;
    h->prof_on = false; h->prof_n = 0;
}

int codae_destroy(codae_handle h) {
    if (h) profile_release(h);
    if (h && h->graph_exec) { (void)hipGraphExecDestroy(h->graph_exec); h->graph_exec = nullptr; }
    if (h && h->side) {
        (void)hipStreamSynchronize(h->side);
        for (int i = 0; i < CODAE_MAX_DACT; ++i) if (h->ev_ready[i]) (void)hipEventDestroy(h->ev_ready[i]);
        (void)hipEventDestroy(h->ev_join);
        for (int i = 0; i < CODAE_MAX_DACT; ++i) (void)hipEventDestroy(h->ev_w[i]);
        (void)hipStreamDestroy(h->side);
    }
    if (h && h->dp) (void)codae_dp_destroy(h);
    delete h;
    return CODAE_OK;
}

int codae_profile_begin(codae_handle h, uint32_t class_mask, int32_t max_records) {
    CODAE_REQUIRE(h && max_records > 0 && max_records <= (1 << 20), "codae_profile_begin: bad arguments");
    profile_release(h);
    h->prof_start.resize(max_records); h->prof_stop.resize(max_records); h->prof_kind.assign(max_records, -1); h->prof_count.assign(max_records, 1);
    for (int i = 0; i < max_records; ++i) {
        CODAE_HIP_CHECK(hipEventCreate(&h->prof_start[i]));
        CODAE_HIP_CHECK(hipEventCreate(&h->prof_stop[i]));
    }
    h->prof_mask = class_mask; h->prof_n = 0; h->prof_on = true; h->prof_step = 0;
    return CODAE_OK;
}

int codae_profile_stride(codae_handle h, int32_t every_n_steps) {
    CODAE_REQUIRE(h && every_n_steps >= 1, "codae_profile_stride: bad arguments");
    h->prof_every = every_n_steps;
    return CODAE_OK;
}

int codae_profile_end(codae_handle h, int32_t* kinds, float* ms, int32_t capacity, int32_t* n_out) {
    CODAE_REQUIRE(h && kinds && ms && n_out, "codae_profile_end: null argument");
    h->prof_on = false;
    int n = 0;
    for (int i = 0; i < h->prof_n && n < capacity; ++i) {
        CODAE_HIP_CHECK(hipEventSynchronize(h->prof_stop[i]));
        float t = 0.f;
        CODAE_HIP_CHECK(hipEventElapsedTime(&t, h->prof_start[i], h->prof_stop[i]));
        const int c = h->prof_count[i];
        for (int k = 0; k < c && n < capacity; ++k) { kinds[n] = h->prof_kind[i]; ms[n] = t / (float)c; ++n; }
    }
    *n_out = n;
    profile_release(h);
    return CODAE_OK;
}

int codae_get_sizes(codae_handle h, codae_sizes* out) {
    CODAE_REQUIRE(h && out, "codae_get_sizes: null argument");
    out->n_param = h->n_param;
    out->n_weight = h->prec == CODAE_PREC_BF16 ? h->n_param + (int64_t)64 * h->maxw : 0;
    out->act_bytes = h->act_bytes;
    out->dact_bytes = h->n_dact * h->dact_one;
    out->slab_bytes = 3 * h->slab_bytes;
    out->bias_part_bytes = h->part_floats * 4;
    out->n_scalars = CODAE_S_COUNT;
    return CODAE_OK;
}

int codae_param_offsets(codae_handle h, int32_t layer, int64_t* w_off, int64_t* b_off, int64_t* shadow_off) {
    CODAE_REQUIRE(h && layer >= 0 && layer < h->L, "codae_param_offsets: layer %d", layer);
    if (w_off) *w_off = h->w_off[layer];
    if (b_off) *b_off = h->b_off[layer];
    if (shadow_off) *shadow_off = h->w_off[layer];
    return CODAE_OK;
}

int codae_sync_shadows(codae_handle h, const codae_buffers* b, void* stream) {
    CODAE_REQUIRE(h && b && b->params, "codae_sync_shadows: null argument");
    if (h->tc.tied && !h->tie_pairs.empty()) {
        int rc = launch_tie_mirror(b->params, nullptr, nullptr, h->tie_pairs.data(), (int)h->tie_pairs.size(), (hipStream_t)stream);
        if (rc) return rc;
    }
    if (h->prec != CODAE_PREC_BF16) return CODAE_OK;
    CODAE_REQUIRE(b->shadow_w, "codae_sync_shadows: shadow_w missing");
    int rc = launch_cast_bf16(b->params, reinterpret_cast<bf16_t*>(b->shadow_w), h->n_param, (hipStream_t)stream);
    if (rc) return rc;
    return refresh_transposed(h, b, (hipStream_t)stream);
}

int codae_forward(codae_handle h, const codae_buffers* b, const float* x, float* y, int32_t B, int32_t layer_lo,
                  int32_t layer_hi, int32_t save_for_backward, void* stream) {
    int rc = check_common(h, b, B);
    if (rc) return rc;
    CODAE_REQUIRE(x && y, "codae_forward: null x or y");
    CODAE_REQUIRE(layer_lo >= 0 && layer_lo < layer_hi && layer_hi <= h->L, "codae_forward: layer range [%d, %d)", layer_lo, layer_hi);
    (void)save_for_backward;
    h->drop_live = false;
    hipStream_t s = (hipStream_t)stream;
// ... 39 lines not shown
}

static int run_slot_contrast(codae_handle h, const codae_buffers* b, const codae_hyper* hyper, LossLaunch ll, hipStream_t s) {
    if (!h->contrast_on()) return CODAE_OK;
    const int B = ll.batch->B;
    const int blocks = slot_contrast_blocks(B);
    CODAE_REQUIRE(blocks <= h->loss_part_cap && blocks <= (h->max_rows + 31) / 32,
                  "slot contrast: %d row blocks exceed the partial-sum rows (%d)", blocks, h->loss_part_cap);
    const double rows = hyper->loss_scale_rows > 0.f ? (double)hyper->loss_scale_rows : (double)B;
    const double scale = (double)h->tc.contrast.weight / (rows * (double)h->tc.contrast.n_slots);
    ll.emph = h->tc.emph_on ? &h->tc.emph : nullptr;
    ll.scale = (float)scale;
    int rc;
    {
        ProfScope prof(h, CODAE_K_LOSS, s);
        rc = launch_slot_contrast_prepare(ll.batch->data, ll.batch->io, &h->tc.contrast, ll.step, ll.step_dev, ll.dy_bf16, s, ll.present, ll.n_slots);
    }
    if (rc) return rc;
    {
        ProfScope prof(h, CODAE_K_LOSS, s);
        rc = launch_slot_contrast(ll, &h->tc.contrast, s);
    }
    if (rc) return rc;
    h->parts_pending[h->L - 1] = blocks;
    return launch_slot_contrast_finish(b->scalars, scale, ll.parts, blocks, s);
}

static int run_standalone_loss(codae_handle h, const codae_buffers* b, const codae_batch* batch, const codae_hyper* hyper, const float* y,
                               hipStream_t s) {
    const int L = h->L, blocks = mse_loss_colsum_rows(batch->B);
    const double inv_n = loss_inv_n(hyper, batch);
    codae_emphasis unit{};
    unit.alpha = 1.f; unit.beta = 1.f;
    LossLaunch ll{batch, &h->tc.noise, hyper->step, step_dev(h, b), h->tc.emph_on ? &h->tc.emph : nullptr, h->tc.pres.table, h->tc.pres.n_slots,
                  y, dact_ptr(h, b, L - 1), h->prec == CODAE_PREC_BF16, h->out_ld[L - 1], (float)inv_n, part_ptr(h, b, L - 1), loss_parts_ptr(h, b)};
    const bool weighted = h->recon_on() || h->tc.emph_on || ll.present != nullptr;
    int rc;
    {
        ProfScope prof(h, CODAE_K_LOSS, s);
        if (h->recon_on()) {
            rc = launch_recon_loss(ll, &h->tc.recon, s);
        } else if (weighted) {
            if (!h->tc.emph_on) ll.emph = &unit;
            rc = launch_emph_loss(ll, s);
        } else {
            rc = launch_mse_loss(ll, 1, s);
        }
    }
    if (rc) return rc;
    h->parts_pending[L - 1] = blocks;
    h->norm_scalars_zero = true;
    rc = weighted ? launch_finish_emph_loss(b->scalars, inv_n, s, ll.parts, blocks) : finish_loss(h, b, batch, blocks, s);
    return rc ? rc : run_slot_contrast(h, b, hyper, ll, s);
}

static int forward_loss_impl(codae_handle h, const codae_buffers* b, const codae_batch* batch, const codae_hyper* hyper,
                             float* out_y, void* stream, LossFinish* fold) {
    CODAE_REQUIRE(batch != nullptr, "codae_step_forward_loss: null batch");
    int rc = check_common(h, b, batch->B);
    if (rc) return rc;
    CODAE_REQUIRE(batch->io == h->in[0] && batch->io == h->out[h->L - 1], "batch.io %d does not match the model (%d -> %d)",
                  batch->io, h->in[0], h->out[h->L - 1]);
    CODAE_REQUIRE(b->grads && b->dacts && b->scalars, "codae_step_forward_loss: grads / dacts / scalars missing");
    CODAE_REQUIRE(b->bias_parts, "codae_step_forward_loss: bias_parts missing");
    if (h->prof_on) ++h->prof_step;
    hipStream_t s = (hipStream_t)stream;
    const int B = batch->B, L = h->L;
    const int rows = h->rows_for(B);
    const bool bf = h->prec == CODAE_PREC_BF16;
    h->drop_live = hyper != nullptr && h->tc.drop.on;
    if (h->drop_live) { h->drop_B = B; h->drop_rows = batch->row_idx; h->drop_step = hyper->step; }
    const uint8_t* const pres = h->tc.pres.table;
    const int pres_slots = h->tc.pres.n_slots;
    const bool fuse_loss = bf && hyper != nullptr && out_y == nullptr && !h->cfg.no_fused_loss && h->plain_mse();
    const bool fold_finish = fuse_loss && fold != nullptr && !h->cfg.no_folded_loss_finish;
    {
        ProfScope prof(h, CODAE_K_GATHER, s);
        double* zero_norm = fold_finish ? b->scalars : nullptr;
        if (hyper != nullptr && h->tc.noise.kind != CODAE_NOISE_NONE)
            rc = launch_gather_noise(batch, &h->tc.noise, hyper->step, step_dev(h, b),
                                     act_ptr(h, b, 0), bf, s, h->in_ld[0], nullptr, zero_norm, pres, pres_slots);
        else
            rc = launch_gather_corrupt(batch, act_ptr(h, b, 0), bf, s, h->in_ld[0], zero_norm, pres, pres_slots);
    }
    if (rc) return rc;
    rc = zero_pad_rows(h, act_ptr(h, b, 0), B, rows, h->in_ld[0], s);
    if (rc) return rc;
    float* y = out_y ? out_y : reinterpret_cast<float*>(act_ptr(h, b, L));
    GroupScope fwd_group(h, CODAE_K_GEMM_FWD, s);
    if (h->drop_live) fwd_group.close();
    for (int l = 0; l < L; ++l) {
        const bool last = (l == L - 1);
        if (last && fuse_loss) {
            fwd_group.close();
            GemmBf16 g = layer_fwd_bf16(h, b, l, act_ptr(h, b, l), dact_ptr(h, b, l), h->out_ld[l], false, rows);
            g.colsum_part = part_ptr(h, b, l);
            g.loss.enabled = 1; g.loss.data = batch->data; g.loss.row_idx = batch->row_idx; g.loss.mask_id = batch->mask_id;
            g.loss.mask_to_use = batch->mask_to_use; g.loss.nb_run = batch->nb_run; g.loss.run = batch->run;
            g.loss.table = batch->mask_table; g.loss.io = batch->io; g.loss.B = B; g.loss.inv_n = (float)loss_inv_n(hyper, batch);
            g.loss.parts = loss_parts_ptr(h, b);
            if (b->shadow_wt != nullptr && l >= 1 && !h->cfg.no_wt && !h->cfg.no_prefetch) {
                g.prefetch = reinterpret_cast<const bf16_t*>(b->shadow_wt) + h->w_off[l];
                g.prefetch_bytes = (int64_t)h->in[l] * h->out[l] * 2;
            }
            const int n_loss_parts = gemm_bf16_loss_parts(g);
            CODAE_REQUIRE(n_loss_parts <= h->loss_part_cap, "fused loss: %d workgroups exceed the partial-sum rows (%d)", n_loss_parts, h->loss_part_cap);
            {
                ProfScope prof(h, CODAE_K_LOSS, s);
                rc = gemm_bf16(g, s);
            }
            if (rc) return rc;
            h->parts_pending[l] = gemm_bf16_colsum_rows(g);
            h->norm_scalars_zero = true;
            if (fold_finish) {
                fold->scalars = b->scalars; fold->inv_n = 1.0 / ((double)B * batch->io);
                fold->parts = loss_parts_ptr(h, b); fold->n_parts = n_loss_parts;
                return CODAE_OK;
            }
            return finish_loss(h, b, batch, n_loss_parts, s);
        }
        rc = last ? run_linear(h, b, l, act_ptr(h, b, l), y, true, B, s)
                  : run_linear(h, b, l, act_ptr(h, b, l), act_ptr(h, b, l + 1), false, rows, s);
        if (rc) return rc;
        fwd_group.launched();
        if (drops_layer(h, l)) {
            rc = run_dropout_fwd(h, b, l, s);
            if (rc) return rc;
        }
    }
    fwd_group.close();
    if (hyper != nullptr) {
        rc = zero_pad_rows(h, dact_ptr(h, b, L - 1), B, rows, h->out_ld[L - 1], s);
        if (rc) return rc;
        return run_standalone_loss(h, b, batch, hyper, y, s);
// ... 40 lines not shown
    if (rc) return rc;
    CODAE_REQUIRE(loss == nullptr || loss->kind != CODAE_LOSS_SLOT_COSINE || h->tc.pres.table == nullptr || loss->n_slots == h->tc.pres.n_slots,
                  "codae_set_recon_loss: slot_cosine n_slots %d differs from the presence table's %d", loss->n_slots, h->tc.pres.n_slots);
    codae_recon_loss r{};
    const bool on = loss != nullptr && loss->kind != CODAE_LOSS_MSE;
    if (on) {
        r.kind = loss->kind;
        if (loss->kind == CODAE_LOSS_SMOOTH_L1 || loss->kind == CODAE_LOSS_HUBER) r.param = loss->param;
        if (loss->kind == CODAE_LOSS_SLOT_COSINE) { r.mse_weight = loss->mse_weight; r.n_slots = loss->n_slots; }
    }
    h->tc.recon = r;
    return CODAE_OK;
}

int codae_set_slot_contrast(codae_handle h, const codae_slot_contrast* contrast) {
    CODAE_REQUIRE(h != nullptr, "codae_set_slot_contrast: null handle");
    int rc = check_slot_contrast(contrast, h->out[h->L - 1], h->prec == CODAE_PREC_BF16);
    if (rc) return rc;
    CODAE_REQUIRE(contrast == nullptr || contrast->weight == 0.f || h->tc.pres.table == nullptr ||
                      (contrast->n_slots == h->tc.pres.n_slots && (int64_t)contrast->n_rows <= h->tc.pres.n_rows),
                  "codae_set_slot_contrast: n_slots %d / n_rows %d do not fit the presence table (%d slots, %lld rows)", contrast->n_slots,
                  contrast->n_rows, h->tc.pres.n_slots, (long long)h->tc.pres.n_rows);
    codae_slot_contrast c{};
    const bool on = contrast != nullptr && contrast->weight != 0.f;
    if (on) {
        rc = slot_contrast_warm();
        if (rc) return rc;
        c.n_slots = contrast->n_slots; c.n_neg = contrast->n_neg; c.tau = contrast->tau; c.weight = contrast->weight;
        c.seed = contrast->seed; c.n_rows = contrast->n_rows; c.n_pool = contrast->pool ? contrast->n_pool : 0;
        c.ws_bytes = contrast->ws_bytes; c.pool = contrast->pool; c.item_id = contrast->item_id; c.ws = contrast->ws;
    }
    h->tc.contrast = c;
    return CODAE_OK;
}

int codae_set_slot_presence(codae_handle h, const uint8_t* present, int64_t n_rows, int32_t n_slots) {
    CODAE_REQUIRE(h != nullptr, "codae_set_slot_presence: null handle");
    codae_engine::PresCfg p{};
    if (present != nullptr) {
        int rc = check_presence(present, n_slots, h->out[h->L - 1], "codae_set_slot_presence");
        if (rc) return rc;
        CODAE_REQUIRE(n_rows >= 1, "codae_set_slot_presence: n_rows %lld must be >= 1", (long long)n_rows);
        CODAE_REQUIRE(!(h->recon_on() && h->tc.recon.kind == CODAE_LOSS_SLOT_COSINE) || h->tc.recon.n_slots == n_slots,
                      "codae_set_slot_presence: n_slots %d differs from slot_cosine's %d", n_slots, h->tc.recon.n_slots);
        CODAE_REQUIRE(!h->contrast_on() || (h->tc.contrast.n_slots == n_slots && (int64_t)h->tc.contrast.n_rows <= n_rows),
                      "codae_set_slot_presence: %d slots / %lld rows do not fit the slot contrast (%d slots, %d rows)", n_slots,
                      (long long)n_rows, h->tc.contrast.n_slots, h->tc.contrast.n_rows);
        p.table = present; p.n_rows = n_rows; p.n_slots = n_slots;
    }
    h->tc.pres = p;
    return CODAE_OK;
}

int codae_set_optimizer(codae_handle h, const codae_optimizer* opt) {
    CODAE_REQUIRE(h != nullptr, "codae_set_optimizer: null handle");
    int rc = check_optimizer(opt);
    if (rc) return rc;
    h->tc.opt = optimizer_canonical(opt);
    return CODAE_OK;
}

int codae_set_tied_weights(codae_handle h, int32_t on) {
    CODAE_REQUIRE(h != nullptr, "codae_set_tied_weights: null handle");
    if (on) {
        for (int l = 0; l < h->L / 2; ++l) {
            const int m = h->L - 1 - l;
            if (h->in[l] != h->out[m] || h->out[l] != h->in[m]) {
                set_error("tied weights: layers %d and %d are not mirror images (%d -> %d against %d -> %d)", l, m, h->in[l], h->out[l],
                          h->in[m], h->out[m]);
                return CODAE_E_UNSUPPORTED;
            }
        }
        h->tie_pairs.clear();
        for (int l = 0; l < h->L / 2; ++l) {
            codae_tie_pair p{};
            p.enc_off = h->w_off[l]; p.dec_off = h->w_off[h->L - 1 - l]; p.rows = h->out[l]; p.cols = h->in[l];
            h->tie_pairs.push_back(p);
        }
    }
    h->tc.tied = on ? 1 : 0;
    return CODAE_OK;
}

int codae_graph_captures(codae_handle h) { return h != nullptr ? h->graph_captures : 0; }

int codae_set_hidden_dropout(codae_handle h, const codae_dropout* d) {
    CODAE_REQUIRE(h != nullptr, "codae_set_hidden_dropout: null handle");
    codae_engine::DropCfg c{};
    if (d != nullptr) {
        CODAE_REQUIRE(d->n == h->L - 1, "codae_set_hidden_dropout: %d values for %d hidden outputs (n_layers - 1)", d->n, h->L - 1);
        CODAE_REQUIRE(d->n == 0 || d->p != nullptr, "codae_set_hidden_dropout: null p");
        for (int l = 0; l < d->n; ++l) {
            char who[64];
            snprintf(who, sizeof(who), "codae_set_hidden_dropout: layer %d", l);
            int rc = check_dropout_p(d->p[l], who);
            if (rc) return rc;
        }
        for (int l = 0; l < d->n; ++l) {
            if (!(d->p[l] > 0.f)) continue;
            if (h->act[l] != CODAE_ACT_NONE && h->act[l] != CODAE_ACT_LEAKY) {
                set_error("codae_set_hidden_dropout: layer %d: dropout after activation kind %d is not supported (NONE, RELU and LEAKY only)",
                          l, (int)h->act[l]);
                return CODAE_E_UNSUPPORTED;
            }
            c.p[l] = d->p[l];
            c.on = 1;
// ... 325 lines not shown
```

mui-deepautoencoder_amd/csrc/gemm_bf16_pipe.hip:

```cpp
#include "codae_common.h"
#include <type_traits>

namespace codae {
namespace {

#include "gemm_bf16_halftile.h"

constexpr int TIMELINE_WGS = 4096, TIMELINE_SLOTS = 6;
__device__ unsigned long long g_timeline[TIMELINE_WGS * TIMELINE_SLOTS];

constexpr int PARK_BIAS_BYTES = 1024;
template <int BM, int BN, bool C_F32, int EPI>
constexpr int pipe_smem_bytes() {
    const bool park = BM == 256;
    return 2 * (BM + BN) * 128 + (EPI == 3 ? BM * 8 : 0) + (park ? PARK_BIAS_BYTES : 0) + (park && !C_F32 && (EPI == 0 || EPI == 2 || EPI == 4) ? BM * BN / 8 : 0);
}

template <int BM, int BN, int WM, int WN, int NLB, int A_MODE, int B_MODE, bool C_F32, int DBG = 0, int EPI = 0, int POL = STORE_PLAIN>
__device__ __forceinline__ void gemm_bf16_pipe_tile(const GemmBf16& g, int tiles_n, int tiles_mn, int kt_total, int wg, int nwg,
                                                    char* smem_raw) {
    constexpr int NW = WM * WN;
    constexpr int SM = BM / WM, SN = BN / WN;
    constexpr int AHR = BM / 2, BHR = BN / 2;
    constexpr int TMH = SM / 32, TNH = SN / 32;
// ... 400 lines not shown
#pragma unroll
        for (int nh = 0; nh < 2; ++nh)
#pragma unroll
            for (int nt = 0; nt < TNH; ++nt)
#pragma unroll
                for (int k = 0; k < 4; ++k) {
                    float v = cs[nh][nt][k];
                    v += __shfl_xor(v, 1); v += __shfl_xor(v, 2); v += __shfl_xor(v, 4); v += __shfl_xor(v, 8);
                    cs[nh][nt][k] = v;
                }
        phase_barrier();
        float* red = reinterpret_cast<float*>(smem_raw);
        static_assert((WM * BN + 2 * NW) * 4 <= 2 * BUF, "reduction scratch must fit");
        if (li == 0) {
#pragma unroll
            for (int nh = 0; nh < 2; ++nh)
#pragma unroll
                for (int nt = 0; nt < TNH; ++nt) {
                    const int jl = nh * BHR + wc * (SN / 2) + 16 * nt + g4;
#pragma unroll
                    for (int k = 0; k < 4; ++k) red[wr * BN + jl + k] = cs[nh][nt][k];
                }
        }
        float* wsum = red + WM * BN;
        if (lane == 0) { wsum[2 * w] = sq; wsum[2 * w + 1] = sqp; }
        phase_barrier();
        if (threadIdx.x == 0) {
            float a = 0.f, b2 = 0.f;
            for (int ww = 0; ww < NW; ++ww) { a += wsum[2 * ww]; b2 += wsum[2 * ww + 1]; }
            L.parts[2 * bid] = (double)a;
            L.parts[2 * bid + 1] = masked ? (double)b2 : 0.0;
        }
        if (g.colsum_part != nullptr) {
            for (int col = threadIdx.x; col < BN; col += NT) {
                float sum = 0.f;
#pragma unroll
                for (int r = 0; r < WM; ++r) sum += red[r * BN + col];
                if (j0 + col < g.N) g.colsum_part[(int64_t)tm * g.N + j0 + col] = sum;
            }
        }
        consume_prefetch();
        return;
    }
    if constexpr (!C_F32 && !dbg_nostore) {
        constexpr int NT = 64 * NW;
        constexpr int PITCH = BN * 2 + 16;
        static_assert(BM * PITCH <= 2 * BUF, "output tile must fit in the staging buffers");
        const float floor_v = g.relu ? 0.f : -__builtin_inff();
        constexpr int CH = BN / 8, RL = NT / CH;
        constexpr int ITER = (BM + RL - 1) / RL;
        const int c = threadIdx.x % CH, rl = threadIdx.x / CH;
        const int j = j0 + c * 8;
        const int jc = j < g.N ? j : 0;
        const bool bit_mask = EPI == 4 || (EPI != 1 && g.relu_bits != nullptr);
        uint8_t hb[ITER];
        if constexpr (EPI != 1 && !PARK_BITS) {
            if (bit_mask) {
#pragma unroll
                for (int it = 0; it < ITER; ++it) {
                    const int r = rl + it * RL;
                    const bool ok = rl < RL && j < g.N && r < BM && i0 + r < g.M;
                    hb[it] = g.relu_bits[(int64_t)(ok ? i0 + r : 0) * g.ld_bits + (ok ? (jc >> 3) : 0)];
                }
            }
        }
        float4 bjs[2][TNH];
#pragma unroll
        for (int nh = 0; nh < 2; ++nh)
#pragma unroll
            for (int nt = 0; nt < TNH; ++nt) bjs[nh][nt] = bias4(nh * BHR + wc * (SN / 2) + 16 * nt + g4);
#pragma unroll
        for (int nh = 0; nh < 2; ++nh)
#pragma unroll
            for (int nt = 0; nt < TNH; ++nt) {
                const int jl = nh * BHR + wc * (SN / 2) + 16 * nt + g4;
                const float4 bj = bjs[nh][nt];
#pragma unroll
                for (int mh = 0; mh < 2; ++mh)
#pragma unroll
                    for (int mt = 0; mt < TMH; ++mt) {
                        const int il = mh * AHR + wr * (SM / 2) + 16 * mt + li;
                        const f32x4 a = acc[mh][mt][nh][nt];
                        const float v0 = clamp_below(a[0] + bj.x, floor_v), v1 = clamp_below(a[1] + bj.y, floor_v);
                        const float v2 = clamp_below(a[2] + bj.z, floor_v), v3 = clamp_below(a[3] + bj.w, floor_v);
                        u32x2 o;
                        o[0] = pack_bf16x2(v0, v1);
                        o[1] = pack_bf16x2(v2, v3);
                        *reinterpret_cast<__attribute__((address_space(3))) u32x2*>(smem + il * PITCH + jl * 2) = o;
                    }
            }
        phase_barrier();
        float cs[8] = {0.f, 0.f, 0.f, 0.f, 0.f, 0.f, 0.f, 0.f};
        {
            bf16_t* Cb = reinterpret_cast<bf16_t*>(g.C);
            const TileStore<POL> out(Cb + (int64_t)i0 * g.ldc);
            const bool relu_mask = EPI != 1 && !bit_mask && g.relu_src != nullptr;
            constexpr int MASK_NONE = 0, MASK_BITS = 1, MASK_ACT = 2;
            auto write_out = [&](auto kind_tag) {
                constexpr int KIND = decltype(kind_tag)::value;
                uint4 hv[ITER];
                if constexpr (KIND == MASK_ACT) {
#pragma unroll
                    for (int it = 0; it < ITER; ++it) {
                        const int r = rl + it * RL;
                        const bool ok = rl < RL && j < g.N && r < BM && i0 + r < g.M;
                        hv[it] = *reinterpret_cast<const uint4*>(g.relu_src + (int64_t)(ok ? i0 + r : 0) * g.ld_relu + jc);
                    }
                }
                if constexpr (KIND == MASK_BITS && PARK_BITS) {
#pragma unroll
                    for (int it = 0; it < ITER; ++it) {
                        const int r = rl + it * RL;
                        const bool ok = rl < RL && r < BM;
                        hb[it] = *reinterpret_cast<const __attribute__((address_space(3))) uint8_t*>(smem + BITS_OFF + (ok ? r * (BN / 8) + c : 0));
                    }
                }
#pragma unroll
                for (int it = 0; it < ITER; ++it) {
                    const int r = rl + it * RL;
                    const bool ok = rl < RL && j < g.N && r < BM && i0 + r < g.M;
                    const u32x4 lv = *reinterpret_cast<const __attribute__((address_space(3))) u32x4*>(smem + (ok ? r : 0) * PITCH + c * 16);
                    uint4 v = make_uint4(lv[0], lv[1], lv[2], lv[3]);
                    if constexpr (KIND == MASK_BITS) {
                        const uint32_t hbv = hb[it];
                        auto keepb = [](uint32_t val, uint32_t b2) -> uint32_t {
                            return val & (((b2 & 1u) ? 0x0000ffffu : 0u) | ((b2 & 2u) ? 0xffff0000u : 0u));
                        };
                        v.x = keepb(v.x, hbv); v.y = keepb(v.y, hbv >> 2); v.z = keepb(v.z, hbv >> 4); v.w = keepb(v.w, hbv >> 6);
                    } else if constexpr (KIND == MASK_ACT) {
                        const uint4 h = hv[it];
                        auto keep = [](uint32_t val, uint32_t hh) -> uint32_t {
                            const uint32_t lo = ((hh & 0x8000u) == 0 && (hh & 0x7fffu) != 0) ? 0x0000ffffu : 0u;
                            const uint32_t hi = ((hh & 0x80000000u) == 0 && (hh & 0x7fff0000u) != 0) ? 0xffff0000u : 0u;
                            return val & (lo | hi);
                        };
                        v.x = keep(v.x, h.x); v.y = keep(v.y, h.y); v.z = keep(v.z, h.z); v.w = keep(v.w, h.w);
                    }
                    if constexpr (EPI == 1) {
                        if (g.relu_bits_out != nullptr) {
                            auto pos = [](uint32_t w2) -> uint32_t {
                                const uint32_t t = (w2 & 0x7fff7fffu) + 0x7fff7fffu;
                                return ((t >> 15) & 1u) | ((t >> 30) & 2u);
                            };
                            const uint32_t b0 = ok ? (pos(v.x) | (pos(v.y) << 2) | (pos(v.z) << 4) | (pos(v.w) << 6)) : 0u;
                            const uint32_t b1 = (uint32_t)__builtin_amdgcn_update_dpp(0, (int)b0, 0x39, 0xf, 0xf, true);
                            const uint32_t b2 = (uint32_t)__builtin_amdgcn_update_dpp(0, (int)b0, 0x4e, 0xf, 0xf, true);
                            const uint32_t b3 = (uint32_t)__builtin_amdgcn_update_dpp(0, (int)b0, 0x93, 0xf, 0xf, true);
                            if (ok && (c & 3) == 0)
                                *reinterpret_cast<uint32_t*>(g.relu_bits_out + (int64_t)(i0 + r) * g.ld_bits + (j >> 3)) = b0 | (b1 << 8) | (b2 << 16) | (b3 << 24);
                        }
                    }
                    if (ok) {
                        out.store16(Cb + (int64_t)(i0 + r) * g.ldc + j, (uint32_t)(r * (int)g.ldc + j) * 2u, (u32x4){v.x, v.y, v.z, v.w});
                        if (EPI != 1 && g.colsum_part != nullptr) {
                            cs[0] += bf16_to_f32((bf16_t)(v.x & 0xffff)); cs[1] += bf16_to_f32((bf16_t)(v.x >> 16));
                            cs[2] += bf16_to_f32((bf16_t)(v.y & 0xffff)); cs[3] += bf16_to_f32((bf16_t)(v.y >> 16));
                            cs[4] += bf16_to_f32((bf16_t)(v.z & 0xffff)); cs[5] += bf16_to_f32((bf16_t)(v.z >> 16));
                            cs[6] += bf16_to_f32((bf16_t)(v.w & 0xffff)); cs[7] += bf16_to_f32((bf16_t)(v.w >> 16));
                        }
                    }
                }
            };
            if constexpr (EPI == 1) write_out(std::integral_constant<int, MASK_NONE>{});
            else if constexpr (EPI == 4) write_out(std::integral_constant<int, MASK_BITS>{});
            else if (bit_mask) write_out(std::integral_constant<int, MASK_BITS>{});
            else if (relu_mask) write_out(std::integral_constant<int, MASK_ACT>{});
            else write_out(std::integral_constant<int, MASK_NONE>{});
        }
        stamp(3);
        if constexpr (dbg_time) { wait_vmcnt<0>(); stamp(4); }
        if (EPI != 1 && g.colsum_part != nullptr) {
            phase_barrier();
            float* red = reinterpret_cast<float*>(smem_raw);
            static_assert(RL * BN * 4 <= 2 * BUF, "reduction scratch must fit");
            if (rl < RL) {
#pragma unroll
                for (int k = 0; k < 8; ++k) red[rl * BN + c * 8 + k] = cs[k];
            }
            phase_barrier();
            for (int col = threadIdx.x; col < BN; col += NT) {
                float sum = 0.f;
                for (int r = 0; r < RL; ++r) sum += red[r * BN + col];
                if (j0 + col < g.N) g.colsum_part[(int64_t)tm * g.N + j0 + col] = sum;
            }
        }
        consume_prefetch();
        return;
    }
    if constexpr (C_F32) {
        constexpr int NT = 64 * NW;
        constexpr int HR = AHR;
        constexpr int PITCH = BN * 4 + 16;
        static_assert(HR * PITCH <= 2 * BUF, "fp32 half tile must fit in the staging buffers");
        constexpr int CH = BN / 4, RL = NT / CH;
        float* Cf = reinterpret_cast<float*>(g.C);
        if (g.split_k > 1) Cf += (int64_t)z * g.M * g.ldc;
        const float floor_v = g.relu ? 0.f : -__builtin_inff();
        const int c = threadIdx.x % CH, rl = threadIdx.x / CH;
        const int j = j0 + c * 4;
        float sq = 0.f;
        float4 bjs[2][TNH];
#pragma unroll
        for (int nh = 0; nh < 2; ++nh)
#pragma unroll
            for (int nt = 0; nt < TNH; ++nt) bjs[nh][nt] = bias4(nh * BHR + wc * (SN / 2) + 16 * nt + g4);
#pragma unroll
        for (int hh = 0; hh < 2; ++hh) {
#pragma unroll
            for (int nh = 0; nh < 2; ++nh)
#pragma unroll
                for (int nt = 0; nt < TNH; ++nt) {
                    const int jl = nh * BHR + wc * (SN / 2) + 16 * nt + g4;
                    const float4 bj = bjs[nh][nt];
#pragma unroll
                    for (int mt = 0; mt < TMH; ++mt) {
                        const int il = wr * (SM / 2) + 16 * mt + li;
                        const f32x4 a = acc[hh][mt][nh][nt];
                        f32x4 v;
                        v[0] = clamp_below(a[0] + bj.x, floor_v); v[1] = clamp_below(a[1] + bj.y, floor_v);
                        v[2] = clamp_below(a[2] + bj.z, floor_v); v[3] = clamp_below(a[3] + bj.w, floor_v);
                        *reinterpret_cast<__attribute__((address_space(3))) f32x4*>(smem + il * PITCH + jl * 4) = v;
                    }
                }
            phase_barrier();
            constexpr int ITER = (HR + RL - 1) / RL;
            const TileStore<POL> out(Cf + (int64_t)(i0 + hh * HR) * g.ldc);
#pragma unroll
            for (int it = 0; it < ITER; ++it) {
                const int r = rl + it * RL;
                const bool ok = rl < RL && j < g.N && r < HR && i0 + hh * HR + r < g.M;
                const f32x4 v = *reinterpret_cast<const __attribute__((address_space(3))) f32x4*>(smem + (ok ? r : 0) * PITCH + c * 16);
                if (ok) {
                    out.store16(Cf + (int64_t)(i0 + hh * HR + r) * g.ldc + j, (uint32_t)(r * (int)g.ldc + j) * 4u, __builtin_bit_cast(u32x4, v));
                    sq += v[0] * v[0] + v[1] * v[1] + v[2] * v[2] + v[3] * v[3];
                }
            }
            phase_barrier();
        }
        if (g.sumsq_slots != nullptr) {
#pragma unroll
            for (int o = 32; o > 0; o >>= 1) sq += __shfl_xor(sq, o);
            float* red = reinterpret_cast<float*>(smem_raw);
            if (lane == 0) red[w] = sq;
            phase_barrier();
            if (threadIdx.x == 0) {
                float t = 0.f;
                for (int ww = 0; ww < NW; ++ww) t += red[ww];
                atomicAdd(g.sumsq_slots + (wg & (CODAE_S_N_SLOTS - 1)), (double)t);
            }
        }
    }
}

template <int BM, int BN, int WM, int WN, int NLB, int A_MODE, int B_MODE, bool C_F32, int DBG = 0, int EPI = 0, int POL = STORE_PLAIN>
__global__ __launch_bounds__(64 * WM * WN, (WM * WN + 3) / 4)
void gemm_bf16_pipe_kernel(GemmBf16 g, int tiles_n, int tiles_mn, int kt_total) {
    __shared__ __attribute__((aligned(16))) char smem_raw[pipe_smem_bytes<BM, BN, C_F32, EPI>()];
    gemm_bf16_pipe_tile<BM, BN, WM, WN, NLB, A_MODE, B_MODE, C_F32, DBG, EPI, POL>(g, tiles_n, tiles_mn, kt_total, blockIdx.x, gridDim.x, smem_raw);
}

template <int POL>
__global__ __launch_bounds__(512, 2) void gemm_bf16_pipe_grouped_kernel(GemmBf16Group grp) {
    constexpr int BM = 256, BN = 192;
    __shared__ __attribute__((aligned(16))) char smem_raw[pipe_smem_bytes<BM, BN, true, 0>()];
    const int total = grp.wg_begin[grp.n];
    int t = (int)blockIdx.x;
    {
        const int q = total >> 3, r = total & 7, xcd = t & 7;
        t = (xcd < r ? xcd * (q + 1) : r * (q + 1) + (xcd - r) * q) + (t >> 3);
    }
    int j = 0;
    while (j + 1 < grp.n && t >= grp.wg_begin[j + 1]) ++j;
    const GemmBf16& g = grp.g[j];
    const int tiles_m = (g.M + BM - 1) / BM, tiles_n = (g.N + BN - 1) / BN;
    gemm_bf16_pipe_tile<BM, BN, 4, 2, 4, OP_KS, OP_KS, true, 0, 0, POL>(g, tiles_n, tiles_m * tiles_n, g.K / BK, t - grp.wg_begin[j], 0, smem_raw);
}

#define PIPE_LAUNCH(BM, BN, NLB, AM, BMODE, CF, DBG, EP, POL)                                                                    \
    hipLaunchKernelGGL((gemm_bf16_pipe_kernel<BM, BN, 4, 2, NLB, AM, BMODE, CF, DBG, EP, POL>), dim3((unsigned)p.workgroups), dim3(512), 0, s, g, \
                       p.tiles_n, p.tiles_m * p.tiles_n, g.K / BK)

template <int NLB>
int launch_pipe(const GemmBf16& g, const Bf16Plan& p, hipStream_t s) {
    constexpr int BM = 256, BN = 192;
#define LAUNCH(AM, BMODE, CF, EP) \
    do { if (p.store_policy == STORE_WT) PIPE_LAUNCH(BM, BN, NLB, AM, BMODE, CF, 0, EP, STORE_WT); else PIPE_LAUNCH(BM, BN, NLB, AM, BMODE, CF, 0, EP, STORE_PLAIN); } while (0)
#define LAUNCH_BF16(AM, BMODE) do { if (p.epi == 2) LAUNCH(AM, BMODE, false, 2); else LAUNCH(AM, BMODE, false, 1); } while (0)
    const bool bits = p.epi == 2 && g.relu_bits != nullptr;
    if (p.dbg == 64) PIPE_LAUNCH(BM, BN, NLB, OP_KC, OP_KC, false, 64, 2, STORE_PLAIN);
    else if (p.epi == 3) LAUNCH(OP_KC, OP_KC, false, 3);
    else if (g.a_mode == OP_KC && g.b_mode == OP_KC) { if (g.c_f32) LAUNCH(OP_KC, OP_KC, true, 0); else if (bits) LAUNCH(OP_KC, OP_KC, false, 4); else LAUNCH_BF16(OP_KC, OP_KC); }
    else if (g.a_mode == OP_KC && g.b_mode == OP_KS) { if (g.c_f32) LAUNCH(OP_KC, OP_KS, true, 0); else LAUNCH_BF16(OP_KC, OP_KS); }
    else if (g.a_mode == OP_KS && g.b_mode == OP_KS) { if (g.c_f32) LAUNCH(OP_KS, OP_KS, true, 0); else LAUNCH_BF16(OP_KS, OP_KS); }
    else { set_error("gemm_bf16: operand mode combination not built"); return CODAE_E_UNSUPPORTED; }
#undef LAUNCH_BF16
#undef LAUNCH
    CODAE_LAUNCH_CHECK();
    return CODAE_OK;
}

template <int DBG>
int launch_dbg(const GemmBf16& g, const Bf16Plan& p, hipStream_t s) {
    if (DBG == 8 && p.store_policy == STORE_WT) PIPE_LAUNCH(256, 192, 4, OP_KC, OP_KC, false, 8, 0, STORE_WT);
    else PIPE_LAUNCH(256, 192, 4, OP_KC, OP_KC, false, DBG, 0, STORE_PLAIN);
    CODAE_LAUNCH_CHECK();
    return CODAE_OK;
}

int launch_pipe_mid(const GemmBf16& g, const Bf16Plan& p, hipStream_t s) {
    const bool wt = p.store_policy == STORE_WT;
    if (p.epi == 2) { if (wt) PIPE_LAUNCH(128, 192, 4, OP_KC, OP_KC, false, 0, 2, STORE_WT); else PIPE_LAUNCH(128, 192, 4, OP_KC, OP_KC, false, 0, 2, STORE_PLAIN); }
    else { if (wt) PIPE_LAUNCH(128, 192, 4, OP_KC, OP_KC, false, 0, 1, STORE_WT); else PIPE_LAUNCH(128, 192, 4, OP_KC, OP_KC, false, 0, 1, STORE_PLAIN); }
    CODAE_LAUNCH_CHECK();
    return CODAE_OK;
}

}

int gemm_bf16_pipe_grouped(GemmBf16Group& grp, hipStream_t s) {
    CODAE_REQUIRE(grp.n >= 1 && grp.n <= CODAE_GROUP_MAX, "gemm_bf16_pipe_grouped: %d GEMMs", grp.n);
    int total = 0;
    int64_t out_bytes = 0;
    for (int j = 0; j < grp.n; ++j) out_bytes += (int64_t)grp.g[j].M * grp.g[j].N * 4;
    bool all_wt = store_policy_for(out_bytes) == STORE_WT;
    for (int j = 0; j < grp.n; ++j) {
        const GemmBf16& g = grp.g[j];
        CODAE_REQUIRE(g.a_mode == OP_KS && g.b_mode == OP_KS && g.c_f32 && g.split_k == 1 && g.K % BK == 0 && g.K >= BK && g.M % 8 == 0 &&
                          g.N % 8 == 0 && g.M >= 8 && g.N >= 8 && !g.loss.enabled && g.relu_src == nullptr && g.colsum_part == nullptr &&
                          g.bias == nullptr && !g.relu && (g.lda % 8) == 0 && (g.ldb % 8) == 0 && (g.ldc % 4) == 0,
                      "gemm_bf16_pipe_grouped: GEMM %d is not a plain unsplit weight-gradient form", j);
        CODAE_REQUIRE((int64_t)g.K * g.lda * 2 < (int64_t)1 << 32 && (int64_t)g.K * g.ldb * 2 < (int64_t)1 << 32,
                      "gemm_bf16_pipe_grouped: operand larger than 4 GiB");
        CODAE_REQUIRE((reinterpret_cast<uintptr_t>(g.A) & 15) == 0 && (reinterpret_cast<uintptr_t>(g.B) & 15) == 0 &&
                          (reinterpret_cast<uintptr_t>(g.C) & 15) == 0, "gemm_bf16_pipe_grouped: operands must be 16-byte aligned");
        if (g.store_policy != STORE_WT || g.ldc >= ((int64_t)1 << 20)) all_wt = false;
        grp.wg_begin[j] = total;
        total += tile_count(g.M, g.N, TILE_256x192);
    }
    grp.wg_begin[grp.n] = total;
    if (all_wt) hipLaunchKernelGGL(gemm_bf16_pipe_grouped_kernel<STORE_WT>, dim3(total), dim3(512), 0, s, grp);
    else hipLaunchKernelGGL(gemm_bf16_pipe_grouped_kernel<STORE_PLAIN>, dim3(total), dim3(512), 0, s, grp);
    CODAE_LAUNCH_CHECK();
    return CODAE_OK;
}

int gemm_bf16_pipe(const GemmBf16& g_in, const Bf16Plan& p, hipStream_t s) {
    CODAE_REQUIRE((int64_t)(g_in.a_mode == OP_KC ? g_in.M : g_in.K) * g_in.lda * 2 < (int64_t)1 << 32 &&
                      (int64_t)(g_in.b_mode == OP_KC ? g_in.N : g_in.K) * g_in.ldb * 2 < (int64_t)1 << 32,
                  "gemm_bf16: operand larger than 4 GiB");
    GemmBf16 g = g_in;
    g.store_policy = p.store_policy;
    if (p.family == BF16_PIPELINED_ABL) {
        g.dbg = p.dbg;
        if (p.epi == 3) {
            PIPE_LAUNCH(256, 192, 6, OP_KC, OP_KC, false, 8, 3, STORE_PLAIN);
            CODAE_LAUNCH_CHECK();
            return CODAE_OK;
        }
        switch (p.dbg) {
            case 1: return launch_dbg<1>(g, p, s);
            case 2: return launch_dbg<2>(g, p, s);
            case 3: return launch_dbg<3>(g, p, s);
            case 4: return launch_dbg<4>(g, p, s);
            case 5: return launch_dbg<5>(g, p, s);
            case 6: return launch_dbg<6>(g, p, s);
            case 7: return launch_dbg<7>(g, p, s);
            case 8: return launch_dbg<8>(g, p, s);
            case 9: return launch_dbg<9>(g, p, s);
            case 10: return launch_dbg<10>(g, p, s);
            case 16: return launch_dbg<16>(g, p, s);
            case 32: return launch_dbg<32>(g, p, s);
            default: set_error("gemm_bf16: ablation build %d is not instantiated", p.dbg); return CODAE_E_UNSUPPORTED;
        }
    }
    if (p.loader == 7) return launch_pipe_mid(g, p, s);
    return p.loader == 6 ? launch_pipe<4>(g, p, s) : launch_pipe<6>(g, p, s);
}
#undef PIPE_LAUNCH

int gemm_bf16_timeline(unsigned long long* host_out, int n_wg) {
    CODAE_REQUIRE(host_out && n_wg > 0 && n_wg <= TIMELINE_WGS, "timeline: bad args");
    CODAE_HIP_CHECK(hipMemcpyFromSymbol(host_out, HIP_SYMBOL(g_timeline), (size_t)n_wg * TIMELINE_SLOTS * sizeof(unsigned long long)));
    return CODAE_OK;
}

}
```

mui-deepautoencoder_amd/csrc/primitives.hip:

```cpp
#include "layer_gemm.h"

using namespace codae;

namespace {

int linear_f32(const char* who, const float* x, const float* W, const float* bias, float* y, int M, int N, int K, int relu, int act,
               const float* p, hipStream_t s) {
    CODAE_REQUIRE(x && W && y, "%s: null operand", who);
    GemmF32 g = fwd_gemm_f32(x, W, y, M, N, K, bias);
    set_activation(g, relu, act, p);
    return gemm_f32(g, s);
}

int dgrad_f32(const char* who, const float* dy, const float* W, const float* src, float* dx, int M, int N, int K, int act, const float* p,
              hipStream_t s) {
    CODAE_REQUIRE(dy && W && dx, "%s: null operand", who);
    GemmF32 g = dgrad_gemm_f32(dy, W, dx, M, N, K);
    g.relu_src = src; g.ld_relu = K;
    set_activation(g, 0, act, p);
    return gemm_f32(g, s);
}

int linear_bf16(const char* who, const void* x, const void* W, const float* bias, void* y, int y_f32, int M, int N, int K, int relu,
                int act, const float* p, hipStream_t s) {
// ... 221 lines not shown
    return linear_bf16("codae_linear_act_bf16", x, W, bias, y, y_f32, M, N, K, 0, act, p, (hipStream_t)stream);
}

int codae_dgrad_act_bf16(const void* dy, const void* W, const void* act_src, void* dx, float* db_prev, float* db_ws, int32_t M,
                         int32_t N, int32_t K, int32_t act, float p0, float p1, float p2, void* stream) {
    CODAE_REQUIRE(act >= CODAE_ACT_NONE && act <= CODAE_ACT_HARDSIGMOID, "codae_dgrad_act_bf16: activation kind %d", act);
    if (act == CODAE_ACT_NONE || act_src == nullptr) return codae_dgrad_bf16(dy, W, nullptr, dx, db_prev, db_ws, M, N, K, stream);
    const float p[3] = {p0, p1, p2};
    return dgrad_bf16("codae_dgrad_act_bf16", dy, W, act_src, dx, db_prev, db_ws, M, N, K, act, p, (hipStream_t)stream);
}

int codae_wgrad_bf16(const void* dy, const void* x, float* dW, void* slabs, int64_t slab_bytes, int32_t M, int32_t N,
                     int32_t K, void* stream) {
    CODAE_REQUIRE(dy && x && dW, "codae_wgrad_bf16: null operand");
    CODAE_REQUIRE(M % 64 == 0, "codae_wgrad_bf16: batch rows %d must be a multiple of 64 (pad with zero rows)", M);
    int S = choose_split_k(N, K, M);
    while (S > 1 && (slabs == nullptr || (int64_t)S * N * K * 4 > slab_bytes)) --S;
    GemmBf16 g = wgrad_gemm_bf16(dy, N, x, K, S > 1 ? slabs : (void*)dW, M, N, K);
    g.split_k = S;
    int rc = gemm_bf16(g, (hipStream_t)stream);
    if (rc) return rc;
    if (S > 1) return launch_reduce_slabs(reinterpret_cast<const float*>(slabs), S, (int64_t)N * K, dW, (int64_t)N * K, nullptr, (hipStream_t)stream);
    return CODAE_OK;
}

int codae_debug_gemm_bf16_plan(const int32_t* desc, int32_t* out, int32_t capacity) {
    CODAE_REQUIRE(desc && out && capacity >= CODAE_GEMM_PLAN_FIELDS, "codae_debug_gemm_bf16_plan: needs room for %d fields", CODAE_GEMM_PLAN_FIELDS);
    GemmBf16 g{};
    g.a_mode = desc[0]; g.b_mode = desc[1]; g.c_f32 = desc[2]; g.M = desc[3]; g.N = desc[4]; g.K = desc[5]; g.split_k = desc[6];
    g.act = desc[7]; g.loss.enabled = desc[8]; g.coscheduled = desc[10]; g.store_policy = desc[11]; g.ldc = desc[12];
    if (desc[11] < 0) g.store_policy = store_policy_for((int64_t)g.M * g.N * (g.c_f32 ? 4 : 2));
    static float some_rows;
    if (desc[9]) g.colsum_part = &some_rows;
    CODAE_REQUIRE(gemm_bf16_supported(g.M, g.N, g.K) && g.split_k >= 1, "codae_debug_gemm_bf16_plan: unsupported shape M=%d N=%d K=%d", g.M, g.N, g.K);
    const Bf16Plan p = gemm_bf16_plan(g);
    const int32_t fields[CODAE_GEMM_PLAN_FIELDS] = {p.family, p.bm, p.bn, p.stages, p.loader, p.epi, p.dbg, p.act, p.store_policy, p.tiles_m, p.tiles_n,
                                                    (int32_t)p.workgroups, gemm_bf16_colsum_rows(g), g.loss.enabled ? gemm_bf16_loss_parts(g) : 0,
                                                    gemm_bf16_takes_relu_bits(g.M, g.N) ? 1 : 0};
    for (int i = 0; i < CODAE_GEMM_PLAN_FIELDS; ++i) out[i] = fields[i];
    return CODAE_OK;
}

int codae_debug_gemm_timeline(uint64_t* host_out, int32_t n_wg) {
    return gemm_bf16_timeline(reinterpret_cast<unsigned long long*>(host_out), n_wg);
}

int codae_transpose_bf16(const void* src, void* dst, int32_t rows, int32_t cols, void* stream) {
    CODAE_REQUIRE(src && dst && rows > 0 && cols > 0, "transpose: bad args");
    const int64_t off = 0;
    return launch_transpose_bf16(reinterpret_cast<const bf16_t*>(src), reinterpret_cast<bf16_t*>(dst), 1, &off, &rows, &cols,
                                 (hipStream_t)stream);
}

int codae_cast_f32_to_bf16(const float* src, void* dst, int64_t n, void* stream) {
    return launch_cast_bf16(src, reinterpret_cast<bf16_t*>(dst), n, (hipStream_t)stream);
}

}
```

Before: 7.097 million samples/s.

## Gather from a cached bf16 dataset image and fold bias-finish into grouped wgrad

Adds a one-time bf16 copy of the fp32 training dataset and a new gather/corrupt kernel that reads bf16 rows directly. This halves input gather traffic and removes the per-step fp32-to-bf16 conversion. Bias-gradient finishing and the loss-scalar reduction are appended as extra workgroups to the grouped wgrad GEMM launch, with arguments passed through the kernarg segment, which saves a separate kernel launch. A specialised unmasked epilogue variant (EPI 5) is also added for bf16 outputs with no activation mask. The trade-offs are extra device memory for the dataset image, a stale image if the data changes without a refresh, and a larger kernel-argument block.

```diff
diff --git a/include/codae_hip.h b/include/codae_hip.h
--- a/include/codae_hip.h
+++ b/include/codae_hip.h
@@ -226,6 +226,7 @@
 int codae_set_slot_contrast(codae_handle h, const codae_slot_contrast* contrast);
 int codae_set_optimizer(codae_handle h, const codae_optimizer* opt);
 int codae_set_slot_presence(codae_handle h, const uint8_t* present, int64_t n_rows, int32_t n_slots);
+int codae_set_dataset_image(codae_handle h, const float* data, const void* image_bf16, int64_t n_rows, int32_t io);
 int codae_set_tied_weights(codae_handle h, int32_t on);
 int codae_graph_captures(codae_handle h);
 int codae_eval_step(codae_handle h, const codae_buffers* bufs, const codae_batch* batch, float* out_y,
@@ -358,6 +359,8 @@
 #define CODAE_GEMM_PLAN_FIELDS 15
 int codae_debug_gemm_bf16_plan(const int32_t* desc, int32_t* out, int32_t capacity);
 int codae_cast_f32_to_bf16(const float* src, void* dst, int64_t n, void* stream);
+int codae_corrupt_batch_image(const codae_batch* batch, const void* image_bf16, const uint8_t* present, int32_t n_slots, void* out,
+                              int64_t out_ld, void* stream);
 int codae_transpose_bf16(const void* src, void* dst, int32_t rows, int32_t cols, void* stream);
 
 #ifdef __cplusplus
diff --git a/mui-deepautoencoder_amd/codae/hip/__init__.py b/mui-deepautoencoder_amd/codae/hip/__init__.py
--- a/mui-deepautoencoder_amd/codae/hip/__init__.py
+++ b/mui-deepautoencoder_amd/codae/hip/__init__.py
@@ -129,6 +129,7 @@
     "codae_tie_fold": (C.c_int, [_P, C.POINTER(TiePair), _I32, _P]),
     "codae_tie_mirror": (C.c_int, [_P, _P, _P, C.POINTER(TiePair), _I32, _P]),
     "codae_set_slot_presence": (C.c_int, [_P, _P, _I64, _I32]),
+    "codae_set_dataset_image": (C.c_int, [_P, _P, _P, _I64, _I32]),
     "codae_corrupt_batch_present": (C.c_int, [C.POINTER(Batch), C.POINTER(Noise), _I32, _P, _P, _I32, _I64, _P, _I32, _P]),
     "codae_mse_loss_present": (C.c_int, [C.POINTER(Batch), _P, _P, _I32, _I64, _F, _P, _P, _P, _I32, _P]),
     "codae_emph_loss_present": (C.c_int, [C.POINTER(Batch), C.POINTER(Noise), _I32, C.POINTER(Emphasis), _P, _P, _I32, _I64, _F, _P, _P,
@@ -189,6 +190,7 @@
     "codae_linear_act_bf16": (C.c_int, [_P, _P, _P, _P, _I32, _I32, _I32, _I32, _I32, _F, _F, _F, _P]),
     "codae_dgrad_act_bf16": (C.c_int, [_P, _P, _P, _P, _P, _P, _I32, _I32, _I32, _I32, _F, _F, _F, _P]),
     "codae_cast_f32_to_bf16": (C.c_int, [_P, _P, _I64, _P]),
+    "codae_corrupt_batch_image": (C.c_int, [C.POINTER(Batch), _P, _P, _I32, _P, _I64, _P]),
     "codae_debug_gemm_timeline": (C.c_int, [_P, _I32]),
     "codae_debug_gemm_bf16_plan": (C.c_int, [_P, _P, _I32]),
     "codae_transpose_bf16": (C.c_int, [_P, _P, _I32, _I32, _P]),
diff --git a/mui-deepautoencoder_amd/codae/hip/engine.py b/mui-deepautoencoder_amd/codae/hip/engine.py
--- a/mui-deepautoencoder_amd/codae/hip/engine.py
+++ b/mui-deepautoencoder_amd/codae/hip/engine.py
@@ -104,6 +104,7 @@
         self.slot_presence = None
         self._presence_table = None
         self.tied_weights = False
+        self._dataset_image = None
         self.optimizer = None
         self.adam_vmax = None
         self.step_count = 0
@@ -299,6 +300,20 @@
         check(self._lib.codae_set_slot_presence(self._h, ptr(table), int(table.shape[0]) if n_rows is None else int(n_rows),
                                                 int(table.shape[1]) if n_slots is None else int(n_slots)))
 
+    def set_dataset_image(self, data):
+        if data is None or self.precision != PREC_BF16:
+            check(self._lib.codae_set_dataset_image(self._h, None, None, 0, 0))
+            self._dataset_image = None
+            return None
+        if data.dtype != torch.float32 or not data.is_contiguous() or data.device != self.device or data.dim() != 2:
+            raise HipError("set_dataset_image: data must be the contiguous fp32 [N, io] dataset on %s" % self.device)
+        with torch.cuda.device(self.device):
+            image = torch.empty(data.shape, dtype=torch.bfloat16, device=self.device)
+            check(self._lib.codae_cast_f32_to_bf16(ptr(data), ptr(image), data.numel(), current_stream()))
+        check(self._lib.codae_set_dataset_image(self._h, ptr(data), ptr(image), int(data.shape[0]), int(data.shape[1])))
+        self._dataset_image = (data, image)
+        return image
+
     def set_optimizer(self, optimizer):
         if optimizer is not None and not hasattr(optimizer, "lr_at"):
             raise HipError("set_optimizer: expected a codae.tool.Optimizer or None, got %r" % (optimizer,))
diff --git a/mui-deepautoencoder_amd/codae/train.py b/mui-deepautoencoder_amd/codae/train.py
--- a/mui-deepautoencoder_amd/codae/train.py
+++ b/mui-deepautoencoder_amd/codae/train.py
@@ -1,3 +1,5 @@
+import os
+
 import torch
 
 from .hostcpu import fit_host_threads, host_cpu_share
@@ -306,7 +308,7 @@
                  max_batch=8192, precision="bf16", device="cuda:0", distributed=False, n_buckets=None, use_graph=False,
                  sharded_update=False, native_dp=False, activation=None, n_slots=None, input_noise=None,
                  loss_emphasis=None, hidden_dropout=None, criterion=None, contrast=None, optimizer=None, presence=None,
-                 tied_weights=None):
+                 tied_weights=None, dataset_image=True):
         from .hip.engine import DaeEngine
         fit_host_threads()
         self.device = torch.device(device)
@@ -314,6 +316,8 @@
         if input_noise is not None:
             self.engine.set_input_noise(input_noise)
         self.data = data.to(device=self.device, dtype=torch.float32).contiguous()
+        self.dataset_image = bool(dataset_image) and not os.environ.get("CODAE_NO_DATASET_IMAGE")
+        self.refresh_dataset_image()
         self.mask_table = None if mask_table_u8 is None else mask_table_u8.to(self.device).contiguous()
         self.mask_to_use = None if mask_to_use_i32 is None else mask_to_use_i32.to(self.device).contiguous()
         self.lr, self.weight_decay, self.clip = lr, weight_decay, clip
@@ -339,6 +343,11 @@
         self._idx_buf = torch.zeros(max_batch, dtype=torch.int32, device=self.device) if self.use_graph else None
         self._mid_buf = torch.zeros(max_batch, dtype=torch.int32, device=self.device) if self.use_graph else None
         self._graph_stream = torch.cuda.Stream(device=self.device) if self.use_graph else None
+
+    def refresh_dataset_image(self):
+        from .hip import PREC_BF16
+        if self.dataset_image and self.engine.precision == PREC_BF16:
+            self.engine.set_dataset_image(self.data)
 
     def set_loss_emphasis(self, emphasis):
         S = None
diff --git a/mui-deepautoencoder_amd/csrc/codae_common.h b/mui-deepautoencoder_amd/csrc/codae_common.h
--- a/mui-deepautoencoder_amd/csrc/codae_common.h
+++ b/mui-deepautoencoder_amd/csrc/codae_common.h
@@ -205,6 +205,8 @@
          no_prefetch = false,
          no_defer_wgrad = false;
     bool no_folded_loss_finish = false;
+    bool no_folded_bias_finish = false;
+    bool no_dataset_image = false;
     int store_policy = -1;
 };
 const EnvToggles& env();
@@ -312,7 +314,8 @@
     int wg_begin[CODAE_GROUP_MAX + 1];
 };
 int gemm_bf16_grouped(GemmBf16Group& grp, hipStream_t s);
-int gemm_bf16_pipe_grouped(GemmBf16Group& grp, hipStream_t s);
+struct BiasFold;
+int gemm_bf16_pipe_grouped(GemmBf16Group& grp, hipStream_t s, const BiasFold* fold = nullptr);
 
 constexpr int CODAE_CHAIN_MAX_WIDTH = 512;
 constexpr int CODAE_CHAIN_MAX_LAYERS = 16;
@@ -340,6 +343,9 @@
 
 int launch_gather_corrupt(const codae_batch* b, void* out, int out_bf16, hipStream_t s, int64_t out_ld = 0, double* zero_norm = nullptr,
                           const uint8_t* present = nullptr, int n_slots = 0);
+bool gather_image_takes(const codae_batch* b, const void* image, const void* out, int64_t out_ld);
+int launch_gather_image(const codae_batch* b, const bf16_t* image, bf16_t* out, hipStream_t s, int64_t out_ld = 0, double* zero_norm = nullptr,
+                        const uint8_t* present = nullptr, int n_slots = 0);
 int check_noise(const codae_noise* noise);
 int launch_gather_noise(const codae_batch* b, const codae_noise* noise, int32_t step, const double* step_dev, void* out,
                         int out_bf16, hipStream_t s, int64_t out_ld = 0, const int32_t* noise_rows = nullptr, double* zero_norm = nullptr,
@@ -417,5 +423,14 @@
 };
 struct LossFinish { double* scalars; double inv_n; const double* parts; int n_parts; };
 int launch_bias_finish(const BiasFinishJobs& jobs, double* sumsq, hipStream_t s, const LossFinish* loss = nullptr);
-
-}
+struct BiasFold {
+    int n;
+    int rows[CODAE_GROUP_MAX], cols[CODAE_GROUP_MAX];
+    int col_begin[CODAE_GROUP_MAX + 1];
+    const float* parts[CODAE_GROUP_MAX];
+    float* out[CODAE_GROUP_MAX];
+    double* sumsq;
+    LossFinish loss;
+};
+
+}
diff --git a/mui-deepautoencoder_amd/csrc/elementwise.hip b/mui-deepautoencoder_amd/csrc/elementwise.hip
--- a/mui-deepautoencoder_amd/csrc/elementwise.hip
+++ b/mui-deepautoencoder_amd/csrc/elementwise.hip
@@ -59,6 +59,50 @@
         uint4 o;
         o.x = pack_bf16x2(v[0], v[1]); o.y = pack_bf16x2(v[2], v[3]);
         o.z = pack_bf16x2(v[4], v[5]); o.w = pack_bf16x2(v[6], v[7]);
+        *reinterpret_cast<uint4*>(out + (int64_t)b * out_ld + c) = o;
+    }
+}
+
+__device__ __forceinline__ uint32_t keep_pair(uint32_t m2) {
+    return ((m2 & 0xffu) ? 0x0000ffffu : 0u) | ((m2 & 0xff00u) ? 0xffff0000u : 0u);
+}
+
+template <bool PRES>
+__global__ __launch_bounds__(NT) void gather_corrupt_image_kernel(const bf16_t* __restrict__ image,
+                                                                  const int32_t* __restrict__ row_idx,
+                                                                  const int32_t* __restrict__ mask_id,
+                                                                  const uint8_t* __restrict__ table, int B, int io,
+                                                                  bf16_t* __restrict__ out,
+                                                                  const int32_t* __restrict__ mask_to_use, int nb_run,
+                                                                  int run, int64_t out_ld, double* zero_norm, PresArgs pa) {
+    zero_norm_scalars(zero_norm);
+    const bool masked = (mask_id != nullptr) || (mask_to_use != nullptr);
+    const int cols = io / 8;
+    const int64_t total = (int64_t)B * cols;
+    for (int64_t e = (int64_t)blockIdx.x * NT + threadIdx.x; e < total; e += (int64_t)gridDim.x * NT) {
+        const int b = (int)(e / cols);
+        const int c = (int)(e - (int64_t)b * cols) * 8;
+        const int64_t src_row = row_idx ? row_idx[b] : b;
+        uint4 keep = make_uint4(~0u, ~0u, ~0u, ~0u);
+        if (masked) {
+            const int id = mask_id ? mask_id[b] : mask_to_use[src_row * nb_run + run];
+            const uint2 m = *reinterpret_cast<const uint2*>(table + (int64_t)id * io + c);
+            keep = make_uint4(keep_pair(m.x), keep_pair(m.x >> 16), keep_pair(m.y), keep_pair(m.y >> 16));
+        }
+        if constexpr (PRES) {
+            int sl[8];
+            slots_of<8>(c, pa.E, sl);
+            const uint32_t pb = present_bits<8>(pa, src_row, sl);
+            keep.x &= ((pb & 1u) ? 0x0000ffffu : 0u) | ((pb & 2u) ? 0xffff0000u : 0u);
+            keep.y &= ((pb & 4u) ? 0x0000ffffu : 0u) | ((pb & 8u) ? 0xffff0000u : 0u);
+            keep.z &= ((pb & 16u) ? 0x0000ffffu : 0u) | ((pb & 32u) ? 0xffff0000u : 0u);
+            keep.w &= ((pb & 64u) ? 0x0000ffffu : 0u) | ((pb & 128u) ? 0xffff0000u : 0u);
+        }
+        uint4 o = make_uint4(0u, 0u, 0u, 0u);
+        if ((keep.x | keep.y | keep.z | keep.w) != 0u) {
+            const uint4 x = *reinterpret_cast<const uint4*>(image + src_row * io + c);
+            o = make_uint4(x.x & keep.x, x.y & keep.y, x.z & keep.z, x.w & keep.w);
+        }
         *reinterpret_cast<uint4*>(out + (int64_t)b * out_ld + c) = o;
     }
 }
@@ -825,6 +869,37 @@
     else GC(false, false);
 #undef GC
 #undef GCP
+    CODAE_LAUNCH_CHECK();
+    return CODAE_OK;
+}
+
+bool gather_image_takes(const codae_batch* b, const void* image, const void* out, int64_t out_ld) {
+    if (b == nullptr || image == nullptr || out == nullptr || b->io <= 0 || b->io % 8 != 0) return false;
+    if (out_ld <= 0) out_ld = b->io;
+    const bool masked = b->mask_id || b->mask_to_use;
+    return out_ld % 8 == 0 && a16(image) && a16(out) && (!masked || (reinterpret_cast<uintptr_t>(b->mask_table) & 7) == 0);
+}
+
+int launch_gather_image(const codae_batch* b, const bf16_t* image, bf16_t* out, hipStream_t s, int64_t out_ld, double* zero_norm,
+                        const uint8_t* present, int n_slots) {
+    if (out_ld <= 0) out_ld = b ? b->io : 0;
+    CODAE_REQUIRE(b && image && out && b->B > 0 && b->io > 0, "gather_image: bad batch");
+    int prc = check_presence(present, n_slots, b->io, "gather_image");
+    if (prc) return prc;
+    const PresArgs pa{present, n_slots, present ? b->io / n_slots : 0};
+    const bool masked = b->mask_id || b->mask_to_use;
+    CODAE_REQUIRE(!masked || b->mask_table, "gather_image: mask ids without mask_table");
+    CODAE_REQUIRE(!b->mask_to_use || b->mask_id || (b->nb_run > 0 && b->run >= 0 && b->run < b->nb_run),
+                  "gather_image: run %d outside [0, %d)", b->run, b->nb_run);
+    CODAE_REQUIRE(gather_image_takes(b, image, out, out_ld),
+                  "gather_image: io %d and out_ld %lld must be multiples of 8, image and out 16-byte and mask_table 8-byte aligned", b->io,
+                  (long long)out_ld);
+    const int grid = grid_for((int64_t)b->B * (b->io / 8));
+#define GCI(P) hipLaunchKernelGGL((gather_corrupt_image_kernel<P>), dim3(grid), dim3(NT), 0, s, image, b->row_idx, b->mask_id, b->mask_table, \
+                                  b->B, b->io, out, b->mask_to_use, b->nb_run, b->run, out_ld, zero_norm, pa)
+    if (present) GCI(true);
+    else GCI(false);
+#undef GCI
     CODAE_LAUNCH_CHECK();
     return CODAE_OK;
 }
diff --git a/mui-deepautoencoder_amd/csrc/engine.hip b/mui-deepautoencoder_amd/csrc/engine.hip
--- a/mui-deepautoencoder_amd/csrc/engine.hip
+++ b/mui-deepautoencoder_amd/csrc/engine.hip
@@ -44,6 +44,8 @@
     e.no_prefetch = getenv("CODAE_NO_PREFETCH") != nullptr;
     e.no_relu_bits = getenv("CODAE_NO_RELU_BITS") != nullptr;
     e.no_folded_loss_finish = getenv("CODAE_NO_FOLDED_LOSS_FINISH") != nullptr;
+    e.no_dataset_image = getenv("CODAE_NO_DATASET_IMAGE") != nullptr;
+    e.no_folded_bias_finish = getenv("CODAE_NO_FOLDED_BIAS_FINISH") != nullptr;
     if (const char* k = getenv("CODAE_STORE_POLICY"))
         e.store_policy = !strcmp(k, "plain") ? STORE_PLAIN : (!strcmp(k, "wt") ? STORE_WT : -1);
     if (const char* k = getenv("CODAE_F32_GEMM")) e.f32_gemm = k[0] == 'n' ? 1 : (k[0] == 'x' ? 2 : 0);
@@ -88,6 +90,7 @@
     bool chain_ok = false;
     struct PresCfg { const uint8_t* table; int64_t n_rows; int32_t n_slots; int32_t reserved; };
     struct DropCfg { float p[64]; uint64_t seed; int32_t on; int32_t reserved; };
+    struct ImageCfg { const float* data; const void* image; int64_t n_rows; int32_t io; int32_t reserved; };
     struct TrainCfg {
         codae_noise noise;
         codae_emphasis emph;
@@ -98,6 +101,7 @@
         DropCfg drop;
         codae_optimizer opt;
         int32_t tied, tied_reserved;
+        ImageCfg img;
     } tc;
     bool recon_on() const { return tc.recon.kind != CODAE_LOSS_MSE; }
     bool contrast_on() const { return tc.contrast.weight != 0.f; }
@@ -232,6 +236,14 @@
     ~GroupScope() { close(); }
 };
 
+void prof_rides_along(codae_engine* e, int kind) {
+    if (e->prof_on && ((e->prof_mask >> kind) & 1u) && (e->prof_step % e->prof_every) == 0 && e->prof_n < (int)e->prof_start.size()) {
+        const int slot = e->prof_n++;
+        e->prof_kind[slot] = kind;
+        e->prof_count[slot] = -1;
+    }
+}
+
 int choose_split_k_f32(int N, int K, int rows) {
     if (env().wgrad_splitk > 0) return env().wgrad_splitk <= rows / 32 ? env().wgrad_splitk : 1;
     if (rows <= 1024) return 1;
@@ -417,7 +429,30 @@
     return gemm_f32x3_grouped(grp, s);
 }
 
-int run_wgrad_deferred(codae_engine* e, const codae_buffers* b, int rows, bool with_norm, hipStream_t s) {
+bool take_bias_fold(codae_engine* e, const codae_buffers* b, bool with_norm, const LossFinish* loss, BiasFold* f) {
+    int n = 0;
+    for (int l = 0; l < e->L; ++l) n += e->parts_pending[l] > 0 ? 1 : 0;
+    if (n == 0 || n > CODAE_GROUP_MAX) return false;
+    *f = BiasFold{};
+    int cols = 0;
+    for (int l = 0; l < e->L; ++l) {
+        if (e->parts_pending[l] <= 0) continue;
+        f->parts[f->n] = part_ptr(e, b, l);
+        f->out[f->n] = b->grads + e->b_off[l];
+        f->rows[f->n] = e->parts_pending[l];
+        f->cols[f->n] = e->out[l];
+        f->col_begin[f->n] = cols;
+        cols += e->out[l];
+        ++f->n;
+        e->parts_pending[l] = 0;
+    }
+    f->col_begin[f->n] = cols;
+    f->sumsq = with_norm ? b->scalars + CODAE_S_GRAD_SQ : nullptr;
+    if (loss != nullptr) f->loss = *loss;
+    return true;
+}
+
+int run_wgrad_deferred(codae_engine* e, const codae_buffers* b, int rows, bool with_norm, hipStream_t s, const BiasFold* fold = nullptr) {
     GemmBf16Group grp{};
     grp.n = 0;
     for (int l = e->L - 1; l >= 0; --l) {
@@ -427,7 +462,7 @@
     }
     ProfScope prof(e, CODAE_K_GEMM_WGRAD, s);
     prof.counts_as(grp.n);
-    return gemm_bf16_pipe_grouped(grp, s);
+    return gemm_bf16_pipe_grouped(grp, s, fold);
 }
 
 int gemm_f32_small(codae_engine* e, const codae_buffers* b, const GemmF32& g, hipStream_t s) {
@@ -643,9 +678,13 @@
             rc = run_dgrad(h, b, l, rows, false, nullptr, s);
             if (rc) return rc;
         }
+        BiasFold fold;
+        const bool folded = defer == 1 && !h->cfg.no_folded_bias_finish && take_bias_fold(h, b, with_norm, loss, &fold);
         rc = defer == 3 ? run_wgrad_deferred_f32(h, b, rows, s)
-                        : (defer == 1 ? run_wgrad_deferred(h, b, rows, with_norm, s) : run_wgrad_grouped(h, b, rows, with_norm, s));
-        if (rc) return rc;
+                        : (defer == 1 ? run_wgrad_deferred(h, b, rows, with_norm, s, folded ? &fold : nullptr)
+                                      : run_wgrad_grouped(h, b, rows, with_norm, s));
+        if (rc) return rc;
+        if (folded) { prof_rides_along(h, CODAE_K_BIAS_FINISH); return CODAE_OK; }
         return finish_bias(h, b, s, with_norm, loss);
     }
     bool* w_pending = h->w_pending;
@@ -893,6 +932,7 @@
     h->prof_on = false;
     int n = 0;
     for (int i = 0; i < h->prof_n && n < capacity; ++i) {
+        if (h->prof_count[i] < 0) { kinds[n] = h->prof_kind[i]; ms[n] = 0.f; ++n; continue; }
         CODAE_HIP_CHECK(hipEventSynchronize(h->prof_stop[i]));
         float t = 0.f;
         CODAE_HIP_CHECK(hipEventElapsedTime(&t, h->prof_start[i], h->prof_stop[i]));
@@ -1038,6 +1078,12 @@
     h->norm_scalars_zero = true;
     rc = weighted ? launch_finish_emph_loss(b->scalars, inv_n, s, ll.parts, blocks) : finish_loss(h, b, batch, blocks, s);
     return rc ? rc : run_slot_contrast(h, b, hyper, ll, s);
+}
+
+static bool gathers_from_image(codae_handle h, const codae_batch* batch, const void* out) {
+    const codae_engine::ImageCfg& im = h->tc.img;
+    return h->prec == CODAE_PREC_BF16 && !h->cfg.no_dataset_image && im.image != nullptr && batch->data == im.data && batch->io == im.io &&
+           gather_image_takes(batch, im.image, out, h->in_ld[0]);
 }
 
 static int forward_loss_impl(codae_handle h, const codae_buffers* b, const codae_batch* batch, const codae_hyper* hyper,
@@ -1066,6 +1112,9 @@
         if (hyper != nullptr && h->tc.noise.kind != CODAE_NOISE_NONE)
             rc = launch_gather_noise(batch, &h->tc.noise, hyper->step, step_dev(h, b),
                                      act_ptr(h, b, 0), bf, s, h->in_ld[0], nullptr, zero_norm, pres, pres_slots);
+        else if (gathers_from_image(h, batch, act_ptr(h, b, 0)))
+            rc = launch_gather_image(batch, reinterpret_cast<const bf16_t*>(h->tc.img.image), reinterpret_cast<bf16_t*>(act_ptr(h, b, 0)), s,
+                                     h->in_ld[0], zero_norm, pres, pres_slots);
         else
             rc = launch_gather_corrupt(batch, act_ptr(h, b, 0), bf, s, h->in_ld[0], zero_norm, pres, pres_slots);
     }
@@ -1212,6 +1261,20 @@
     return CODAE_OK;
 }
 
+int codae_set_dataset_image(codae_handle h, const float* data, const void* image_bf16, int64_t n_rows, int32_t io) {
+    CODAE_REQUIRE(h != nullptr, "codae_set_dataset_image: null handle");
+    codae_engine::ImageCfg im{};
+    if (image_bf16 != nullptr) {
+        CODAE_REQUIRE(data != nullptr, "codae_set_dataset_image: an image without the dataset it was cast from");
+        CODAE_REQUIRE(n_rows >= 1, "codae_set_dataset_image: n_rows %lld must be >= 1", (long long)n_rows);
+        CODAE_REQUIRE(io == h->in[0], "codae_set_dataset_image: io %d does not match the model (%d)", io, h->in[0]);
+        CODAE_REQUIRE((reinterpret_cast<uintptr_t>(image_bf16) & 15) == 0, "codae_set_dataset_image: the image must be 16-byte aligned");
+        im.data = data; im.image = image_bf16; im.n_rows = n_rows; im.io = io;
+    }
+    h->tc.img = im;
+    return CODAE_OK;
+}
+
 int codae_set_optimizer(codae_handle h, const codae_optimizer* opt) {
     CODAE_REQUIRE(h != nullptr, "codae_set_optimizer: null handle");
     int rc = check_optimizer(opt);
diff --git a/mui-deepautoencoder_amd/csrc/gemm_bf16_pipe.hip b/mui-deepautoencoder_amd/csrc/gemm_bf16_pipe.hip
--- a/mui-deepautoencoder_amd/csrc/gemm_bf16_pipe.hip
+++ b/mui-deepautoencoder_amd/csrc/gemm_bf16_pipe.hip
@@ -476,9 +476,9 @@
         const int c = threadIdx.x % CH, rl = threadIdx.x / CH;
         const int j = j0 + c * 8;
         const int jc = j < g.N ? j : 0;
-        const bool bit_mask = EPI == 4 || (EPI != 1 && g.relu_bits != nullptr);
+        const bool bit_mask = EPI == 4 || (EPI != 1 && EPI != 5 && g.relu_bits != nullptr);
         uint8_t hb[ITER];
-        if constexpr (EPI != 1 && !PARK_BITS) {
+        if constexpr (EPI != 1 && EPI != 5 && !PARK_BITS) {
             if (bit_mask) {
 #pragma unroll
                 for (int it = 0; it < ITER; ++it) {
@@ -518,7 +518,7 @@
         {
             bf16_t* Cb = reinterpret_cast<bf16_t*>(g.C);
             const TileStore<POL> out(Cb + (int64_t)i0 * g.ldc);
-            const bool relu_mask = EPI != 1 && !bit_mask && g.relu_src != nullptr;
+            const bool relu_mask = EPI != 1 && EPI != 5 && !bit_mask && g.relu_src != nullptr;
             constexpr int MASK_NONE = 0, MASK_BITS = 1, MASK_ACT = 2;
             auto write_out = [&](auto kind_tag) {
                 constexpr int KIND = decltype(kind_tag)::value;
@@ -585,7 +585,7 @@
                     }
                 }
             };
-            if constexpr (EPI == 1) write_out(std::integral_constant<int, MASK_NONE>{});
+            if constexpr (EPI == 1 || EPI == 5) write_out(std::integral_constant<int, MASK_NONE>{});
             else if constexpr (EPI == 4) write_out(std::integral_constant<int, MASK_BITS>{});
             else if (bit_mask) write_out(std::integral_constant<int, MASK_BITS>{});
             else if (relu_mask) write_out(std::integral_constant<int, MASK_ACT>{});
@@ -683,10 +683,89 @@
     gemm_bf16_pipe_tile<BM, BN, WM, WN, NLB, A_MODE, B_MODE, C_F32, DBG, EPI, POL>(g, tiles_n, tiles_mn, kt_total, blockIdx.x, gridDim.x, smem_raw);
 }
 
+typedef const __attribute__((address_space(4))) BiasFold* FoldArgs;
+__device__ __attribute__((noinline)) void grouped_bias_finish(FoldArgs f, int fb, int n_fb, char* smem_raw) {
+    constexpr int NT = 256;
+    const int tl = threadIdx.x & (NT - 1), half = threadIdx.x >> 8;
+    if (f->loss.scalars != nullptr && fb == n_fb - 1) {
+        double* lred = reinterpret_cast<double*>(smem_raw);
+        double a = 0.0, b = 0.0;
+        if (half == 0) {
+            const double* parts = f->loss.parts;
+            for (int i = tl; i < f->loss.n_parts; i += NT) { a += parts[2 * i]; b += parts[2 * i + 1]; }
+            lred[tl] = a; lred[NT + tl] = b;
+        }
+        __syncthreads();
+        for (int o = NT / 2; o > 0; o >>= 1) {
+            if (half == 0 && tl < o) { lred[tl] += lred[tl + o]; lred[NT + tl] += lred[NT + tl + o]; }
+            __syncthreads();
+        }
+        if (threadIdx.x == 0) {
+            double* sc = f->loss.scalars;
+            sc[CODAE_S_SQ_FULL] += lred[0];
+            sc[CODAE_S_SQ_PARTIAL] += lred[NT];
+            sc[CODAE_S_LAST_LOSS] = lred[0] * f->loss.inv_n;
+            sc[CODAE_S_STEP_SQ] = 0.0;
+        }
+        return;
+    }
+    const int n = f->n, total = f->col_begin[n];
+    const int vb = 2 * fb + half;
+    const int gc = vb * NT + tl;
+    float sq = 0.f;
+    if (gc < total) {
+        int j = 0;
+        while (j + 1 < n && gc >= f->col_begin[j + 1]) ++j;
+        const int c = gc - f->col_begin[j];
+        const int N = f->cols[j], R = f->rows[j];
+        const float* p = f->parts[j] + c;
+        float s = 0.f;
+        int r = 0;
+        for (; r + 32 <= R; r += 32) {
+            float v[32];
+#pragma unroll
+            for (int u = 0; u < 32; ++u) v[u] = p[(int64_t)(r + u) * N];
+#pragma unroll
+            for (int u = 0; u < 32; ++u) s += v[u];
+        }
+        for (; r + 8 <= R; r += 8) {
+            float v[8];
+#pragma unroll
+            for (int u = 0; u < 8; ++u) v[u] = p[(int64_t)(r + u) * N];
+#pragma unroll
+            for (int u = 0; u < 8; ++u) s += v[u];
+        }
+        for (; r < R; ++r) s += p[(int64_t)r * N];
+        f->out[j][c] = s;
+        sq = s * s;
+    }
+    if (f->sumsq != nullptr) {
+#pragma unroll
+        for (int o = 32; o > 0; o >>= 1) sq += __shfl_xor(sq, o);
+        float* red = reinterpret_cast<float*>(smem_raw);
+        if ((threadIdx.x & 63) == 0) red[threadIdx.x >> 6] = sq;
+        __syncthreads();
+        if (tl == 0 && vb * NT < total) {
+            const float bsq = red[4 * half] + red[4 * half + 1] + red[4 * half + 2] + red[4 * half + 3];
+            atomicAdd(f->sumsq + (CODAE_S_GRAD_SQ_SLOTS - CODAE_S_GRAD_SQ) + (vb & (CODAE_S_N_SLOTS - 1)), (double)bsq);
+        }
+    }
+}
+inline int bias_fold_workgroups(const BiasFold& f) {
+    return f.n > 0 ? ceil_div(ceil_div(f.col_begin[f.n], 256), 2) + (f.loss.scalars != nullptr ? 1 : 0) : 0;
+}
+constexpr size_t GROUPED_FOLD_OFFSET = (sizeof(GemmBf16Group) + alignof(BiasFold) - 1) / alignof(BiasFold) * alignof(BiasFold);
+static_assert(GROUPED_FOLD_OFFSET + sizeof(BiasFold) <= 6144, "grouped launch: kernel-argument block over its budget");
+
 template <int POL>
-__global__ __launch_bounds__(512, 2) void gemm_bf16_pipe_grouped_kernel(GemmBf16Group grp) {
+__global__ __launch_bounds__(512, 2) void gemm_bf16_pipe_grouped_kernel(GemmBf16Group grp, BiasFold fold_by_value) {
     constexpr int BM = 256, BN = 192;
     __shared__ __attribute__((aligned(16))) char smem_raw[pipe_smem_bytes<BM, BN, true, 0>()];
+    if ((int)blockIdx.x >= grp.wg_begin[grp.n]) {
+        const FoldArgs f = (FoldArgs)((const __attribute__((address_space(4))) char*)__builtin_amdgcn_kernarg_segment_ptr() + GROUPED_FOLD_OFFSET);
+        grouped_bias_finish(f, (int)blockIdx.x - grp.wg_begin[grp.n], (int)gridDim.x - grp.wg_begin[grp.n], smem_raw);
+        return;
+    }
     const int total = grp.wg_begin[grp.n];
     int t = (int)blockIdx.x;
     {
@@ -711,10 +790,11 @@
     do { if (p.store_policy == STORE_WT) PIPE_LAUNCH(BM, BN, NLB, AM, BMODE, CF, 0, EP, STORE_WT); else PIPE_LAUNCH(BM, BN, NLB, AM, BMODE, CF, 0, EP, STORE_PLAIN); } while (0)
 #define LAUNCH_BF16(AM, BMODE) do { if (p.epi == 2) LAUNCH(AM, BMODE, false, 2); else LAUNCH(AM, BMODE, false, 1); } while (0)
     const bool bits = p.epi == 2 && g.relu_bits != nullptr;
+    const bool unmasked = p.epi == 2 && g.relu_bits == nullptr && g.relu_src == nullptr;
     if (p.dbg == 64) PIPE_LAUNCH(BM, BN, NLB, OP_KC, OP_KC, false, 64, 2, STORE_PLAIN);
     else if (p.epi == 3) LAUNCH(OP_KC, OP_KC, false, 3);
-    else if (g.a_mode == OP_KC && g.b_mode == OP_KC) { if (g.c_f32) LAUNCH(OP_KC, OP_KC, true, 0); else if (bits) LAUNCH(OP_KC, OP_KC, false, 4); else LAUNCH_BF16(OP_KC, OP_KC); }
-    else if (g.a_mode == OP_KC && g.b_mode == OP_KS) { if (g.c_f32) LAUNCH(OP_KC, OP_KS, true, 0); else LAUNCH_BF16(OP_KC, OP_KS); }
+    else if (g.a_mode == OP_KC && g.b_mode == OP_KC) { if (g.c_f32) LAUNCH(OP_KC, OP_KC, true, 0); else if (bits) LAUNCH(OP_KC, OP_KC, false, 4); else if (unmasked) LAUNCH(OP_KC, OP_KC, false, 5); else LAUNCH_BF16(OP_KC, OP_KC); }
+    else if (g.a_mode == OP_KC && g.b_mode == OP_KS) { if (g.c_f32) LAUNCH(OP_KC, OP_KS, true, 0); else if (unmasked) LAUNCH(OP_KC, OP_KS, false, 5); else LAUNCH_BF16(OP_KC, OP_KS); }
     else if (g.a_mode == OP_KS && g.b_mode == OP_KS) { if (g.c_f32) LAUNCH(OP_KS, OP_KS, true, 0); else LAUNCH_BF16(OP_KS, OP_KS); }
     else { set_error("gemm_bf16: operand mode combination not built"); return CODAE_E_UNSUPPORTED; }
 #undef LAUNCH_BF16
@@ -741,7 +821,7 @@
 
 }
 
-int gemm_bf16_pipe_grouped(GemmBf16Group& grp, hipStream_t s) {
+int gemm_bf16_pipe_grouped(GemmBf16Group& grp, hipStream_t s, const BiasFold* fold) {
     CODAE_REQUIRE(grp.n >= 1 && grp.n <= CODAE_GROUP_MAX, "gemm_bf16_pipe_grouped: %d GEMMs", grp.n);
     int total = 0;
     int64_t out_bytes = 0;
@@ -762,8 +842,15 @@
         total += tile_count(g.M, g.N, TILE_256x192);
     }
     grp.wg_begin[grp.n] = total;
-    if (all_wt) hipLaunchKernelGGL(gemm_bf16_pipe_grouped_kernel<STORE_WT>, dim3(total), dim3(512), 0, s, grp);
-    else hipLaunchKernelGGL(gemm_bf16_pipe_grouped_kernel<STORE_PLAIN>, dim3(total), dim3(512), 0, s, grp);
+    BiasFold f{};
+    if (fold != nullptr) {
+        f = *fold;
+        CODAE_REQUIRE(f.n >= 1 && f.n <= CODAE_GROUP_MAX && f.col_begin[f.n] > 0, "gemm_bf16_pipe_grouped: %d bias-finish jobs", f.n);
+        CODAE_REQUIRE(f.loss.scalars == nullptr || (f.loss.parts != nullptr && f.loss.n_parts > 0), "gemm_bf16_pipe_grouped: bad loss block");
+    }
+    const int grid = total + bias_fold_workgroups(f);
+    if (all_wt) hipLaunchKernelGGL(gemm_bf16_pipe_grouped_kernel<STORE_WT>, dim3(grid), dim3(512), 0, s, grp, f);
+    else hipLaunchKernelGGL(gemm_bf16_pipe_grouped_kernel<STORE_PLAIN>, dim3(grid), dim3(512), 0, s, grp, f);
     CODAE_LAUNCH_CHECK();
     return CODAE_OK;
 }
diff --git a/mui-deepautoencoder_amd/csrc/primitives.hip b/mui-deepautoencoder_amd/csrc/primitives.hip
--- a/mui-deepautoencoder_amd/csrc/primitives.hip
+++ b/mui-deepautoencoder_amd/csrc/primitives.hip
@@ -297,6 +297,12 @@
                                  (hipStream_t)stream);
 }
 
+int codae_corrupt_batch_image(const codae_batch* batch, const void* image_bf16, const uint8_t* present, int32_t n_slots, void* out,
+                              int64_t out_ld, void* stream) {
+    return launch_gather_image(batch, reinterpret_cast<const bf16_t*>(image_bf16), reinterpret_cast<bf16_t*>(out), (hipStream_t)stream, out_ld,
+                               nullptr, present, n_slots);
+}
+
 int codae_cast_f32_to_bf16(const float* src, void* dst, int64_t n, void* stream) {
     return launch_cast_bf16(src, reinterpret_cast<bf16_t*>(dst), n, (hipStream_t)stream);
 }
```

Result: faster. 7.195 million samples/s, median of 6 (+1.4%).
